# rongzhao-zhang/EfficientQ

Measured on AMD Instinct MI355X. Metric: ptq_calibration_throughput, higher is better.
Workload: dtype i8xi8->i32 (exact) for the Gram systems and per-iteration loss convs of the layers with quantised input, f32/f64 elsewhere

## Files before the change

### efficientq_amd/_lib.py

```python
from __future__ import annotations

import ctypes as C
import os

import torch

_HERE = os.path.dirname(os.path.abspath(__file__))
LIB_PATH = os.path.join(_HERE, "libeffq_hip.so")

EFFQ_OK = 0
_ERR_NAMES = {1: "EFFQ_ERR_ARG", 2: "EFFQ_ERR_HIP", 3: "EFFQ_ERR_WORKSPACE", 4: "EFFQ_ERR_NO_DEVICE",
              5: "EFFQ_ERR_NOT_CONVERGED"}


class EffqError(RuntimeError):
    pass


class Geom(C.Structure):
    _fields_ = [(n, C.c_int32) for n in
                ("N", "C1", "C2", "D", "H", "W", "KD", "KH", "KW", "SD", "SH", "SW", "PD", "PH", "PW")]

    def out_dims(self):
        return ((self.D + 2 * self.PD - self.KD) // self.SD + 1,
                (self.H + 2 * self.PH - self.KH) // self.SH + 1,
                (self.W + 2 * self.PW - self.KW) // self.SW + 1)


class FpState(C.Structure):
    _fields_ = [("alpha", C.c_double), ("alpha_prev", C.c_double), ("sums", C.c_double * 2),
                ("iters", C.c_int32), ("done", C.c_int32)]


FP_STATE_BYTES = C.sizeof(FpState)

_P, _SZ, _I, _F, _D, _LL = C.c_void_p, C.c_size_t, C.c_int, C.c_float, C.c_double, C.c_longlong
_GP = C.POINTER(Geom)
_IP = C.POINTER(C.c_int)
_LLP = C.POINTER(C.c_longlong)


class AdmmRunArgs(C.Structure):
    _fields_ = [("A0", C.c_void_p), ("B0", C.c_void_p), ("W0", C.c_void_p), ("b0", C.c_void_p),
                ("c2", C.c_int32), ("n", C.c_int32), ("has_bias", C.c_int32), ("w_levels", C.c_int32),
                ("iters", C.c_int32), ("rho_period", C.c_int32),
                ("rho", C.c_double), ("rho_max", C.c_double), ("eta", C.c_double), ("tol", C.c_double),
                ("geom", Geom), ("loss_kind", C.c_int32), ("act_levels", C.c_int32),
                ("xq", C.c_void_p), ("xidx", C.c_void_p), ("y_fp", C.c_void_p), ("act_alpha_dev", C.c_void_p),
                ("dual", C.c_void_p), ("wstar", C.c_void_p), ("v", C.c_void_p),
                ("G_ring", C.c_void_p), ("Gq_ring", C.c_void_p), ("b_ring", C.c_void_p), ("state_ring", C.c_void_p),
                ("hist", C.c_void_p), ("err_flag", C.c_void_p),
                ("ainv_pool", C.c_void_p), ("n_ainv", C.c_int32),
                ("prox_ws", C.c_void_p), ("prox_ws_bytes", C.c_size_t),
                ("red_ws", C.c_void_p),
                ("fp_ws", C.c_void_p), ("fp_ws_bytes", C.c_size_t),
                ("fp_pred", C.c_void_p), ("fp_traj_ws", C.c_void_p), ("fp_traj_ws_bytes", C.c_size_t),
                ("inv_ws", C.c_void_p), ("inv_ws_bytes", C.c_size_t),
                ("inv_ws_side", C.c_void_p), ("inv_ws_side_bytes", C.c_size_t),
                ("conv_ws", C.c_void_p), ("conv_ws_bytes", C.c_size_t),
                ("stream_main", C.c_void_p), ("stream_loss", C.c_void_p), ("stream_side", C.c_void_p),
                ("stream_side2", C.c_void_p), ("inv_ws_side2", C.c_void_p), ("inv_ws_side2_bytes", C.c_size_t),
                ("loss_Au", C.c_void_p), ("loss_Bu", C.c_void_p), ("loss_syy", C.c_void_p),
                ("loss_planes", C.c_void_p), ("loss_nplanes", C.c_int32), ("res_ring", C.c_void_p),
                ("channel_wise", C.c_int32), ("alpha_ring", C.c_void_p), ("w_iters_ring", C.c_void_p)]


class ProfRecord(C.Structure):
    _fields_ = [("kind", C.c_int32), ("iter", C.c_int32), ("loss_kind", C.c_int32), ("c2", C.c_int32), ("n", C.c_int32),
                ("geom", Geom), ("ms", C.c_float)]


SIGNATURES = {
    "effq_last_error": (C.c_char_p, []),
    "effq_version": (_I, []),
    "effq_device_count": (_I, [C.POINTER(C.c_int)]),
    "effq_quant_dequant_f32": (_I, [_P, _P, _F, _F, _I, _P, _P, _SZ, _P]),
    "effq_quant_dequant_f64path": (_I, [_P, _P, _D, _D, _I, _P, _P, _P, _SZ, _P]),
    "effq_reduce_ws_bytes": (_SZ, []),
    "effq_abs_sum_f64": (_I, [_P, _SZ, _P, _P, _P]),
    "effq_moments_f64": (_I, [_P, _SZ, _P, _P, _P]),
    "effq_alpha_stats_f64": (_I, [_P, _P, _D, _D, _I, _SZ, _P, _P, _P, _P]),
    "effq_fp_init": (_I, [_P, _P, _P]),
    "effq_fp_update": (_I, [_P, _D, _I, _P]),
    "effq_alpha_fixed_point": (_I, [_P, _SZ, _I, _D, _D, _D, _I, _I, _P, _P, _P]),
    "effq_fp_small_max": (_SZ, []),
    "effq_fixed_point_small": (_I, [_P, _P, _P, _SZ, _I, _D, _D, _D, _I, _P, _P]),
    "effq_fp_coop_max": (_SZ, []),
    "effq_fp_coop_set_spin_limit": (_I, [C.c_uint]),
    "effq_fixed_point_coop": (_I, [_P, _P, _P, _SZ, _I, _D, _D, _D, _I, _P, _P, _P]),
    "effq_fp_bucket_max": (_SZ, []),
    "effq_fp_bucket_ws_bytes": (_SZ, [_SZ]),
    "effq_fixed_point_bucket": (_I, [_P, _P, _P, _SZ, _I, _D, _D, _D, _I, _P, _P, _SZ, _P]),
    "effq_fp_bracket_ws_bytes": (_SZ, [_SZ]),
    "effq_fp_bracket_init": (_I, [_P, _P, _SZ, _I, _I, _P, _SZ, _P]),
    "effq_fp_bracket_run": (_I, [_P, _SZ, _I, _D, _D, _D, _I, _I, _P, _P, _P]),
    "effq_fp_bracket_stats": (_I, [_P, _SZ, _I, _D, _D, _P, _P, _P]),
    "effq_fp_bracket_update": (_I, [_SZ, _I, _D, _D, _D, _I, _P, _P, _P]),
    "effq_fp_traj_max": (_SZ, []),
    "effq_fp_traj_ws_bytes": (_SZ, [_SZ]),
    "effq_spd_inverse_prepare": (_I, [_P]),
    "effq_fp_traj_pred_bytes": (_SZ, []),
    "effq_fixed_point_traj": (_I, [_P, _P, _P, _SZ, _I, _D, _D, _D, _I, _P, _P, _P, _SZ, _P]),
    "effq_fixed_point_bucket_rec": (_I, [_P, _P, _P, _SZ, _I, _D, _D, _D, _I, _P, _P, _SZ, _P, _P]),
    "effq_fixed_point_coop_rec": (_I, [_P, _P, _P, _SZ, _I, _D, _D, _D, _I, _P, _P, _P, _P]),
    "effq_fp_check": (_I, [_P, _P, _P]),
    "effq_fp_channels_max_row": (_I, []),
    "effq_fixed_point_channels": (_I, [_P, _P, _P, _I, _I, _I, _D, _I, _P, _P, _P, _P]),
    "effq_fixed_point_channels_proj": (_I, [_P, _P, _P, _I, _I, _I, _D, _I, _P, _P, _P, _P, _F, _P, _P, _P, _I, _I, _D,
                                            _D, _P]),
    "effq_gram_packed_elems": (_SZ, [_I, _I]),
    "effq_gram_pack": (_I, [_P, _P, _I, _I, _P, _P]),
    "effq_gram_unpack": (_I, [_P, _I, _I, _P, _P, _P]),
    "effq_act_quant_backward": (_I, [_P, _P, _I, _P, _P, _P, _SZ, _P, _P]),
    "effq_att_classes_ws_bytes": (_SZ, []),
    "effq_att_classes": (_I, [_P, _LL, _P, _P, _P, C.POINTER(C.c_int32), _P, _P]),
    "effq_prof_enable": (_I, [_I]),
    "effq_prof_count": (_I, []),
    "effq_prof_read": (_I, [_I, C.POINTER(ProfRecord)]),
    "effq_admm_num_inverses": (_I, [_D, _D, _I, _I]),
    "effq_admm_run": (_I, [C.POINTER(AdmmRunArgs)]),
    "effq_admm_select_best": (_I, [_P, _I, _P, _P, _SZ, _SZ, _P, _P, _P, _P]),
    "effq_gram_ws_bytes": (_SZ, [_GP, _I]),
    "effq_gram_accum": (_I, [_P, _P, _P, _GP, _I, _P, _P, _I, _P, _SZ, _P]),
    "effq_gram_plan_query": (_I, [_GP, _I, _IP, _IP, _IP, _IP, _LLP, _IP, _IP]),
    "effq_gram_i8_supported": (_I, [_GP, _I]),
    "effq_gram_i8_ws_bytes": (_SZ, [_GP, _I]),
    "effq_gram_accum_i8": (_I, [_P, _P, _GP, _I, _P, _I, _P, _P, _P, _I, _LL, _P, _P, _I, _P, _SZ, _P]),
    "effq_gram_accum_i8_unw": (_I, [_P, _P, _GP, _I, _P, _I, _P, _P, _P, _I, _LL, _P, _P, _I, _P, _P, _P, _SZ, _P]),
    "effq_gram_i8_plan_query": (_I, [_GP, _I, _LL, _IP, _IP, _IP, _IP, _IP, _IP]),
    "effq_upsample_trilinear": (_I, [_P, _I, _I, _I, _I, _I, _I, _I, _I, _P, _P]),
    "effq_gram_f64_supported": (_I, [_GP, _I]),
    "effq_gram_f64_ws_bytes": (_SZ, [_GP, _I]),
    "effq_gram_f64": (_I, [_P, _P, _GP, _I, _P, _P, _P, _SZ, _P]),
    "effq_gram_f64_plan_query": (_I, [_GP, _I, _IP, _IP, _IP, _IP]),
    "effq_gram_loss_ws_bytes": (_SZ, [_I]),
    "effq_gram_loss": (_I, [_P, _P, _P, _P, _P, _I, _I, _I, _P, _P, _SZ, _P]),
    "effq_packed_bytes": (_SZ, [_SZ, _I]),
    "effq_pack_levels": (_I, [_P, _SZ, _I, _P, _P]),
    "effq_unpack_levels": (_I, [_P, _SZ, _I, _P, _P]),
    "effq_ainv_ld": (_I, [_I]),
    "effq_fp_bracket_export_words": (_SZ, []),
    "effq_fp_bracket_export": (_I, [_P, _SZ, _P, _P, _SZ, _P]),
    "effq_fp_bracket_rebase": (_I, [_P, _P, _SZ, _P]),
    "effq_fp_bracket_import": (_I, [_P, _SZ, _P, _I, _SZ, _P, _P, _SZ, _P]),
    "effq_admm_uses_traj": (_I, [_SZ, _I]),
    "effq_gram_loss_i8_supported": (_I, [_I, _I, _I, _I]),
    "effq_gram_loss_i8_num_planes": (_I, [C.c_longlong]),
    "effq_gram_loss_i8_planes_bytes": (_SZ, [_I, _I, _I]),
    "effq_gram_loss_i8_prepare": (_I, [_P, _I, _I, _P, _I, _I, _P, _P, _P]),
    "effq_gram_loss_i8_ws_bytes": (_SZ, []),
    "effq_gram_loss_i8": (_I, [_P, _I, _P, _P, _P, _P, _P, _P, _P, _I, _I, _I, _I, _I, _I, _P, _P, _SZ, _P]),
    "effq_spd_inverse_ws_bytes": (_SZ, [_I]),
    "effq_spd_inverse": (_I, [_P, _I, _I, _D, _D, _P, _P, _SZ, _P]),
    "effq_spd_inverse_plan": (_I, [_I, _IP, _IP, _IP]),
    "effq_prox_plan_query": (_I, [_I, _I, _IP, _IP, _IP, _IP]),
    "effq_prox_ws_bytes": (_SZ, [_I, _I]),
    "effq_prox_solve": (_I, [_P, _P, _P, _P, _P, _P, _I, _I, _I, _D, _D, _P, _P, _P, _SZ, _P]),
    "effq_prox_solve_shifted": (_I, [_P, _P, _P, _P, _P, _P, _I, _I, _I, _D, _D, _D, _I, _P, _P, _P, _SZ, _P]),
    "effq_admm_presum": (_I, [_P, _P, _P, _SZ, _P]),
    "effq_admm_project_dual": (_I, [_P, _P, _P, _I, _P, _P, _F, _P, _SZ, _P]),
    "effq_conv_i8_supported": (_I, [_GP, _I, _I]),
    "effq_conv_i8s_supported": (_I, [_GP, _I, _I]),
    "effq_conv_i8s_ws_bytes": (_SZ, [_GP, _I, _I]),
    "conv3d_calib_step_i8s": (_I, [_P, _P, _P, _P, _GP, _P, _I, _P, _I, _I, _P, _P, _SZ, _P]),
    "effq_conv_i8_ws_bytes": (_SZ, [_GP]),
    "conv3d_calib_step_i8": (_I, [_P, _P, _P, _P, _GP, _P, _I, _P, _I, _P, _P, _SZ, _P]),
    "effq_conv_i8_out_supported": (_I, [_GP, _I, _I]),
    "conv3d_quant_forward_i8": (_I, [_P, _P, _P, _P, _P, _GP, _P, _I, _P, _I, _P, _P, _P, _SZ, _P]),
    "effq_conv_ws_bytes": (_SZ, [_GP]),
    "conv3d_quant_calib_step": (_I, [_P, _P, _P, _P, _P, _GP, _P, _I, _P, _P, _P, _SZ, _P]),
    "effq_adam_step": (_I, [_P, _P, _P, _P, _F, _F, _F, _F, _I, _SZ, _P]),
    "effq_window_gather": (_I, [_P, _I, _I, _I, _I, _I, _I, _I, _I, _I, _I, _I, _I, _I, _P, _P]),
    "effq_window_stitch": (_I, [_P, _I, _I, _I, _I, _I, _I, _I, _I, _I, _I, _I, _P, _P]),
    "effq_seg_tallies": (_I, [_P, _P, _I, _LL, _I, _I, _F, _P, _P, _SZ, _P]),
    "effq_seg_labels": (_I, [_P, _I, _I, _LL, _I, _I, _F, _I, _P, _P]),
    "effq_cc_ws_bytes": (_SZ, [_I, _I, _I, _I]),
    "effq_cc_label": (_I, [_P, _I, _I, _I, _I, _I, _P, _P, _P, _SZ, _P]),
    "effq_seg_lesions": (_I, [_P, _P, _I, _I, _I, _I, _I, _I, _F, _I, _P, _P, _SZ, _P]),
    "effq_surf_ws_bytes": (_SZ, [_I, _I, _I, _I]),
    "effq_edt_sq": (_I, [_P, _I, _I, _I, _I, _P, _P, _SZ, _P]),
    "effq_seg_surface": (_I, [_P, _P, _I, _I, _I, _I, _I, _I, _F, _P, _P, _P, _SZ, _P]),
    "effq_surf_mm_ws_bytes": (_SZ, [_I, _I, _I, _I]),
    "effq_edt_sq_mm": (_I, [_P, _I, _I, _I, _I, _F, _F, _F, _P, _P, _SZ, _P]),
    "effq_seg_surface_mm": (_I, [_P, _P, _I, _I, _I, _I, _I, _I, _F, _F, _F, _F, _P, _P, _P, _P, _SZ, _P]),
}

SEG_TALLIES_WS_BYTES = 1024 * 3 * 8 * 4
SEG_TALLIES_MAX_CLASSES = 8
SEG_ARGMAX, SEG_SIGMOID = 0, 1
SEG_FUSE = {None: 0, "agg": 1, "aggressive": 1, "con": 2, "conservative": 2}
SEG_LABEL_RULES = {"argmax": 0, "brats": 1, "rank": 2, "planes": 3}
LESION_CONNECTIVITY = 26
EDT_MAX_LINE = 16382
EDT_MM_MAX_EXTENT = 4096

_lib = None


def load():
    global _lib
    if _lib is not None:
        return _lib
    if not os.path.exists(LIB_PATH):
        raise EffqError(f"{LIB_PATH} is missing: run `python -c 'import __graft_entry__ as g; g.build()'` "
                        f"or `make -C efficientq_amd/csrc` (there is no CPU fallback)")
    lib = C.CDLL(LIB_PATH)
    for name, (res, args) in SIGNATURES.items():
        fn = getattr(lib, name)
        fn.restype, fn.argtypes = res, args
    _lib = lib
    return lib


def check(rc: int, what: str):
    if rc != EFFQ_OK:
        msg = load().effq_last_error().decode(errors="replace")
        raise EffqError(f"{what} failed with {_ERR_NAMES.get(rc, rc)}: {msg}")
```

### efficientq_amd/csrc/admm_run.hip

```cpp
#include <stdlib.h>
#include <algorithm>
#include <vector>
#include "common.h"
#include "internal.h"
#include "project_dual.h"

namespace effq {

struct ProfRec {
  int kind, iter, loss_kind, c2, n;
  effq_geom geom;
  hipEvent_t e0, e1;
};
static thread_local std::vector<ProfRec> g_prof;
static thread_local int g_prof_every = 0;
enum { PROF_PROX = 1, PROF_FIXED_POINT = 2, PROF_PROJECT = 3, PROF_LOSS = 4, PROF_INVERSE = 5, PROF_WAIT = 6 };

struct ProfScope {
  bool on;
  hipStream_t stream;
  ProfRec rec;
  ProfScope(bool enabled, int kind, int iter, const effq_admm_run_args* a, hipStream_t st) : on(enabled), stream(st) {
    if (!on) return;
    rec.kind = kind;
    rec.iter = iter;
    rec.loss_kind = a->loss_kind;
    rec.c2 = a->c2;
    rec.n = a->n;
    rec.geom = a->geom;
    if (hipEventCreate(&rec.e0) != hipSuccess || hipEventCreate(&rec.e1) != hipSuccess) {
      on = false;
      return;
    }
    (void)hipEventRecord(rec.e0, stream);
  }
  void close() {
    if (!on) return;
    (void)hipEventRecord(rec.e1, stream);
    g_prof.push_back(rec);
    on = false;
  }
};

constexpr int ADMM_MAX_RHOS = 16;

struct RhoPlan {
  int count;
  double rho[ADMM_MAX_RHOS];
  int first_iter[ADMM_MAX_RHOS];
  bool shifted_first;
  bool overflow;
};

static RhoPlan plan_rhos(double rho, double rho_max, int iters, int period) {
  RhoPlan p;
  p.count = 0;
  p.overflow = false;
  double r = rho;
  for (int i = 0; i < iters; ++i) {
    if (p.count == 0 || p.rho[p.count - 1] != r) {
      if (p.count == ADMM_MAX_RHOS) {
        p.overflow = true;
        break;
      }
      p.rho[p.count] = r;
      p.first_iter[p.count] = i;
      ++p.count;
    }
    if (i % period == 0) r = (r * 2 <= rho_max) ? r * 2 : rho_max;
  }
  p.shifted_first = p.count > 1 && p.first_iter[1] == 1 && p.rho[1] > p.rho[0];
  return p;
}

static int shift_terms(double rho, double eta, double rho_inv) {
  const double d = rho_inv - rho;
  if (d <= 0) return 1;
  int t = (int)ceil(-26.0 * log(2.0) / log(d / (rho_inv + eta)));
  return t < 2 ? 2 : (t > 64 ? 64 : t);
}

__global__ __launch_bounds__(256) void k_gram_pack(const float* __restrict__ A0, const float* __restrict__ B0, int n, int c2,
                                                   float* __restrict__ buf) {
  const size_t tri = (size_t)n * (n + 1) / 2, nb = (size_t)c2 * n;
  const size_t stride = (size_t)gridDim.x * blockDim.x;
  for (size_t e = (size_t)blockIdx.x * blockDim.x + threadIdx.x; e < (size_t)n * n + nb; e += stride) {
    if (e < (size_t)n * n) {
      const int i = (int)(e / n), j = (int)(e % n);
      if (j >= i) buf[(size_t)i * n - (size_t)i * (i - 1) / 2 + (j - i)] = A0[e];
    } else {
      buf[tri + (e - (size_t)n * n)] = B0[e - (size_t)n * n];
    }
  }
}
__global__ __launch_bounds__(256) void k_gram_unpack(const float* __restrict__ buf, int n, int c2, float* __restrict__ A0,
                                                     float* __restrict__ B0) {
  const size_t tri = (size_t)n * (n + 1) / 2, nb = (size_t)c2 * n;
  const size_t stride = (size_t)gridDim.x * blockDim.x;
  for (size_t e = (size_t)blockIdx.x * blockDim.x + threadIdx.x; e < (size_t)n * n + nb; e += stride) {
    if (e < (size_t)n * n) {
      int i = (int)(e / n), j = (int)(e % n);
      if (j < i) {
        const int t = i;
        i = j;
        j = t;
      }
      A0[e] = buf[(size_t)i * n - (size_t)i * (i - 1) / 2 + (j - i)];
    } else {
      B0[e - (size_t)n * n] = buf[tri + (e - (size_t)n * n)];
    }
  }
}

__global__ __launch_bounds__(256) void k_select_best(const double* __restrict__ hist, int iters,
                                                     const float* __restrict__ G_ring, const float* __restrict__ b_ring,
                                                     size_t nw, size_t nb, float* __restrict__ best_G,
                                                     float* __restrict__ best_b, double* __restrict__ best_out) {
  int bi = 0;
  double bl = hist[0];
  for (int i = 1; i < iters; ++i) {
    const double l = hist[2 * (size_t)i];
    if (l < bl) {
      bl = l;
      bi = i;
    }
  }
  const size_t stride = (size_t)gridDim.x * blockDim.x;
  const size_t t0 = (size_t)blockIdx.x * blockDim.x + threadIdx.x;
  const float* g = G_ring + (size_t)bi * nw;
  for (size_t i = t0; i < nw; i += stride) best_G[i] = g[i];
  if (b_ring != nullptr)
    for (size_t i = t0; i < nb; i += stride) best_b[i] = b_ring[(size_t)bi * nb + i];
  if (t0 == 0) {
    best_out[0] = bl;
    best_out[1] = (double)bi;
  }
}

__global__ __launch_bounds__(256) void k_admm_residuals(const float* __restrict__ wstar, const float* __restrict__ G,
                                                        const float* __restrict__ G0, size_t n, double* __restrict__ res) {
  __shared__ double sh[2][4];
  double a = 0.0, b = 0.0;
  for (size_t i = (size_t)blockIdx.x * blockDim.x + threadIdx.x; i < n; i += (size_t)gridDim.x * blockDim.x) {
    const double p = (double)wstar[i] - (double)G[i], q = (double)G[i] - (double)G0[i];
    a += p * p;
    b += q * q;
  }
  a = wave_sum_f64_dpp(a);
  b = wave_sum_f64_dpp(b);
  const int lane = threadIdx.x & 63, wid = threadIdx.x >> 6;
  if (lane == 0) {
    sh[0][wid] = a;
    sh[1][wid] = b;
  }
  __syncthreads();
  if (threadIdx.x < 2) atomicAdd(res + threadIdx.x, (sh[threadIdx.x][0] + sh[threadIdx.x][1]) + (sh[threadIdx.x][2] + sh[threadIdx.x][3]));
}

struct AdmmPlan {
  int c2, n, has_b;
  size_t nw;
  RhoPlan rhos;
  int first, n_inv;
  size_t ainv_elems;
  bool chan, bucket, traj;
  int traj_after;
  hipStream_t s_main, s_loss, s_side, s_side2;
  bool fork_loss, fork_side, two_sides;
  int side_iter;
  int loss_group;
  float* bm;
  int bm_ld;
};
static int admm_plan(const effq_admm_run_args* a, AdmmPlan* p) {
  EFFQ_CHECK_ARG(a != nullptr);
  EFFQ_CHECK_ARG(a->A0 && a->B0 && a->W0 && a->dual && a->wstar && a->v && a->G_ring && a->state_ring && a->hist &&
                 a->err_flag && a->ainv_pool && a->prox_ws && a->red_ws && a->inv_ws && a->conv_ws && a->y_fp);
  EFFQ_CHECK_ARG(a->c2 > 0 && a->n > 1 && a->iters > 0 && a->rho_period > 0 && a->w_levels >= 2 && a->w_levels <= 256);
  EFFQ_CHECK_ARG((a->has_bias != 0) == (a->b0 != nullptr) && (a->has_bias != 0) == (a->b_ring != nullptr));
  EFFQ_CHECK_ARG((a->loss_kind >= 0 && a->loss_kind <= 2) || a->loss_kind == 4 || a->loss_kind == 5);
  if (a->loss_kind == 4)
    EFFQ_CHECK_ARG(a->loss_Au != nullptr && a->loss_Bu != nullptr && a->loss_syy != nullptr);
  else if (a->loss_kind == 5)
    EFFQ_CHECK_ARG(a->loss_Au != nullptr && a->loss_Bu != nullptr && a->loss_syy != nullptr && a->loss_planes != nullptr &&
                   a->loss_nplanes > 0 && a->Gq_ring != nullptr && a->act_alpha_dev != nullptr &&
                   effq_gram_loss_i8_supported(a->c2, a->n, a->has_bias, a->w_levels));
  else
    EFFQ_CHECK_ARG(a->loss_kind == 0 ? (a->xq != nullptr) : (a->xidx != nullptr && a->Gq_ring != nullptr &&
                                                            a->act_alpha_dev != nullptr));
  p->c2 = a->c2;
  p->n = a->n;
  p->has_b = a->has_bias ? 1 : 0;
  const size_t nw = p->nw = (size_t)p->c2 * (size_t)(p->n - p->has_b);
  EFFQ_CHECK_ARG(nw == (size_t)a->geom.C2 * a->geom.C1 * a->geom.KD * a->geom.KH * a->geom.KW);
  p->chan = a->channel_wise != 0;
  if (p->chan)
    EFFQ_CHECK_ARG((a->loss_kind == 0 || a->loss_kind == 4) && a->alpha_ring != nullptr &&
                   p->n - p->has_b <= effq_fp_channels_max_row());
  if (nw > effq_fp_coop_max()) {
    set_error("admm_run: %zu weights exceed the single-launch fixed points", nw);
    return EFFQ_ERR_ARG;
  }
  constexpr size_t bucket_max = (size_t)1 << 19;
  p->bucket = !p->chan && a->fp_ws != nullptr && a->w_levels <= 16 && nw > 4096 && nw <= bucket_max;
  if (p->bucket && a->fp_ws_bytes < effq_fp_bucket_ws_bytes(nw)) {
    set_error("admm_run: fixed-point workspace %zu < %zu", a->fp_ws_bytes, effq_fp_bucket_ws_bytes(nw));
    return EFFQ_ERR_WORKSPACE;
  }
  p->traj_after = (nw > ((size_t)1 << 20)) ? 30 : 12;
  p->traj = !p->chan && a->fp_pred != nullptr && a->fp_traj_ws != nullptr && effq_admm_uses_traj(nw, a->w_levels) != 0;
  if (p->traj && a->fp_traj_ws_bytes < effq_fp_traj_ws_bytes(nw)) {
    set_error("admm_run: trajectory fixed-point workspace %zu < %zu", a->fp_traj_ws_bytes, effq_fp_traj_ws_bytes(nw));
    return EFFQ_ERR_WORKSPACE;
  }
  p->rhos = plan_rhos(a->rho, a->rho_max, a->iters, a->rho_period);
  EFFQ_CHECK_ARG(!p->rhos.overflow);
  p->first = p->rhos.shifted_first ? 1 : 0;
  p->n_inv = p->rhos.count - p->first;
  EFFQ_CHECK_ARG(a->n_ainv >= p->n_inv);
  p->ainv_elems = (size_t)p->n * (size_t)effq_ainv_ld(p->n);
  p->s_main = as_stream(a->stream_main);
  p->s_loss = a->stream_loss ? as_stream(a->stream_loss) : p->s_main;
  p->s_side = (a->stream_side && a->inv_ws_side) ? as_stream(a->stream_side) : p->s_main;
  p->fork_loss = p->s_loss != p->s_main;
  p->fork_side = p->s_side != p->s_main;
  p->s_side2 = (p->fork_side && a->stream_side2 && a->inv_ws_side2) ? as_stream(a->stream_side2) : p->s_side;
  p->two_sides = p->s_side2 != p->s_side;
  constexpr int SIDE_AFTER_ITERS = 8;
  p->side_iter = p->n_inv <= 1 ? -1 : !p->fork_side ? 0 : std::min(SIDE_AFTER_ITERS, p->rhos.first_iter[p->first + 1] - 1);
  static const int group_gram = getenv("EFFQ_LOSS_GROUP") ? atoi(getenv("EFFQ_LOSS_GROUP")) : 8;
  constexpr int group_conv = 4;
  const int group_size = (a->loss_kind == 4 || a->loss_kind == 5) ? group_gram : group_conv;
  p->loss_group = (p->fork_loss && group_size > 1) ? group_size : 1;
  p->bm = effq_prox_bm(a->prox_ws, p->c2, p->n, &p->bm_ld);
  return EFFQ_OK;
}

struct EventPool {
  std::vector<hipEvent_t>* pool = nullptr;
  size_t used = 0;
  hipError_t open() {
    static thread_local std::vector<std::vector<hipEvent_t>> per_device;
    int dev = 0;
    const hipError_t e = hipGetDevice(&dev);
    if (e == hipSuccess && (int)per_device.size() <= dev) per_device.resize(dev + 1);
    if (e == hipSuccess) pool = &per_device[dev];
    return e;
  }
  hipError_t take(hipEvent_t* ev) {
    if (used == pool->size()) {
      hipEvent_t fresh;
      const hipError_t e = hipEventCreateWithFlags(&fresh, hipEventDisableTiming);
      if (e != hipSuccess) return e;
      pool->push_back(fresh);
    }
    *ev = (*pool)[used++];
    return hipSuccess;
  }
  hipError_t hand_over(hipStream_t from, hipStream_t into, hipEvent_t ev = nullptr) {
    hipError_t e = ev ? hipSuccess : take(&ev);
    if (e == hipSuccess) e = hipEventRecord(ev, from);
    return e == hipSuccess ? hipStreamWaitEvent(into, ev, 0) : e;
  }
};

static int enqueue_later_inverses(const effq_admm_run_args* a, const AdmmPlan& p, EventPool& events, hipEvent_t* ev_inv) {
  for (int r = p.first + 1; r < p.rhos.count; ++r) {
    float* dst = a->ainv_pool + (size_t)(r - p.first) * p.ainv_elems;
    const bool on2 = p.two_sides && ((r - p.first) % 2 == 0);
    hipStream_t sr = on2 ? p.s_side2 : p.s_side;
    void* ws = !p.fork_side ? a->inv_ws : (on2 ? a->inv_ws_side2 : a->inv_ws_side);
    const size_t wsb = !p.fork_side ? a->inv_ws_bytes : (on2 ? a->inv_ws_side2_bytes : a->inv_ws_side_bytes);
    ProfScope ps(g_prof_every > 0, PROF_INVERSE, -1 - r, a, sr);
    const int rc = effq_spd_inverse(a->A0, p.n, p.has_b, p.rhos.rho[r], a->eta, dst, ws, wsb, sr);
    if (rc != EFFQ_OK) return rc;
    ps.close();
    if (p.fork_side) {
      EFFQ_HIP(events.take(&ev_inv[r]));
      EFFQ_HIP(hipEventRecord(ev_inv[r], sr));
    }
  }
  return EFFQ_OK;
}

struct AdmmIter {
  int i;
  double rho, rho_next;
  float dual_div;
  bool use_shift, use_traj, prof;
  bool next_rhs;
  const float* G_prev;
  float *G, *bstar;
  int8_t* Gq;
  effq_fp_state* st;
  const float* parts;
  int parts_n, parts_ld;
};
static AdmmIter admm_iter(const effq_admm_run_args* a, const AdmmPlan& p, int i, double rho, bool use_traj) {
  const bool step = i % a->rho_period == 0, doubles = rho * 2 <= a->rho_max;
  const bool use_shift = p.rhos.shifted_first && i == 0;
  const bool prof = g_prof_every > 0 && !use_shift && (i % g_prof_every) == g_prof_every / 2;
  return AdmmIter{i, rho, !step ? rho : doubles ? rho * 2 : a->rho_max,
                  !step ? 1.0f : doubles ? 2.0f : (float)(a->rho_max / rho), use_shift, use_traj, prof, i + 1 < a->iters,
                  (i == 0) ? a->W0 : a->G_ring + (size_t)(i - 1) * p.nw, a->G_ring + (size_t)i * p.nw,
                  p.has_b ? a->b_ring + (size_t)i * p.c2 : nullptr, a->Gq_ring ? a->Gq_ring + (size_t)i * p.nw : nullptr,
                  a->state_ring + i, nullptr, 1, 0};
}

static int enqueue_prox(const effq_admm_run_args* a, const AdmmPlan& p, AdmmIter* it, const float* Ainv, bool bm_ready) {
  if (!it->use_shift && bm_ready && it->use_traj && p.c2 <= 512)
    return effq_prox_solve_prebuilt_parts(a->B0, Ainv, a->W0, a->b0, it->G_prev, a->dual, p.c2, p.n, p.has_b, it->rho,
                                          a->eta, a->wstar, it->bstar, a->prox_ws, a->prox_ws_bytes, p.s_main,
                                          &it->parts, &it->parts_n, &it->parts_ld);
  if (it->use_shift)
    return effq_prox_solve_shifted(a->B0, a->ainv_pool, a->W0, a->b0, it->G_prev, a->dual, p.c2, p.n, p.has_b, it->rho,
                                   a->eta, p.rhos.rho[1], shift_terms(it->rho, a->eta, p.rhos.rho[1]), a->wstar, it->bstar,
                                   a->prox_ws, a->prox_ws_bytes, p.s_main);
  const auto solve = bm_ready ? effq_prox_solve_prebuilt : effq_prox_solve;
  return solve(a->B0, Ainv, a->W0, a->b0, it->G_prev, a->dual, p.c2, p.n, p.has_b, it->rho, a->eta, a->wstar, it->bstar,
               a->prox_ws, a->prox_ws_bytes, p.s_main);
}

enum class FpKind { channels, traj, bucket, small, coop };
static FpKind fp_kind(const AdmmPlan& p, bool use_traj) {
  if (p.chan) return FpKind::channels;
  if (use_traj) return FpKind::traj;
  if (p.bucket) return FpKind::bucket;
  return p.nw <= effq_fp_small_max() ? FpKind::small : FpKind::coop;
}

static int enqueue_fixed_point(const effq_admm_run_args* a, const AdmmPlan& p, const AdmmIter& it, bool* bm_ready) {
  const int nwrow = p.n - p.has_b;
  const uintptr_t al16 = reinterpret_cast<uintptr_t>(a->v) | reinterpret_cast<uintptr_t>(a->wstar) |
                         reinterpret_cast<uintptr_t>(it.G) | reinterpret_cast<uintptr_t>(a->dual) |
                         (it.next_rhs ? (reinterpret_cast<uintptr_t>(a->W0) | reinterpret_cast<uintptr_t>(p.bm)) : 0);
  const bool vec_ok = (al16 & 15) == 0 && (reinterpret_cast<uintptr_t>(it.Gq) & 3) == 0 && (p.nw % 4) == 0 &&
                      (!it.next_rhs || ((nwrow % 4) == 0 && (p.bm_ld % 4) == 0));
  const FpKind kind = fp_kind(p, it.use_traj);
  const bool fuse_proj = kind == FpKind::channels || (kind == FpKind::small && vec_ok);
  ProjFused pf;
  memset(&pf, 0, sizeof(pf));
  pf.wstar = a->wstar; pf.G = it.G; pf.dual = a->dual; pf.Gq = it.Gq; pf.err_flag = a->err_flag;
  pf.d = 2.0 / (double)(a->w_levels - 1); pf.dual_div = it.dual_div; pf.lm1 = a->w_levels - 1;
  pf.n4 = (unsigned)(p.nw / 4);
  if (it.next_rhs) {
    pf.nx.Bm = p.bm; pf.nx.B0 = a->B0; pf.nx.W0 = a->W0; pf.nx.nwrow = nwrow; pf.nx.n = p.n; pf.nx.ldb = p.bm_ld;
    pf.nx.rho = (float)it.rho_next; pf.nx.eta = (float)a->eta;
  }
  void* rec = p.traj ? a->fp_pred : nullptr;
  const int maxit = 100 * a->w_levels;
  ProfScope p_fp(it.prof, PROF_FIXED_POINT, it.i, a, p.s_main);
  int rc;
  if (kind == FpKind::channels)
    rc = effq_fixed_point_channels_proj(a->wstar, a->dual, a->v, p.c2, nwrow, a->w_levels, a->tol, maxit,
                                        a->alpha_ring + (size_t)it.i * p.c2,
                                        a->w_iters_ring ? a->w_iters_ring + (size_t)it.i * p.c2 : nullptr, a->err_flag,
                                        it.G, it.dual_div, it.next_rhs ? p.bm : nullptr, a->B0, a->W0, p.n, p.bm_ld,
                                        it.rho_next, a->eta, p.s_main);
  else if (kind == FpKind::traj && it.parts != nullptr)
    rc = effq_fixed_point_traj_parts(it.parts, it.parts_n, it.parts_ld, p.c2, nwrow, p.has_b, a->dual, a->wstar, it.bstar,
                                     a->v, a->w_levels, -1.0, 1.0, a->tol, maxit, it.st, a->fp_pred, a->fp_traj_ws,
                                     a->fp_traj_ws_bytes, p.s_main);
  else if (kind == FpKind::traj)
    rc = effq_fixed_point_traj(a->wstar, a->dual, a->v, p.nw, a->w_levels, -1.0, 1.0, a->tol, maxit, it.st, a->fp_pred,
                               a->fp_traj_ws, a->fp_traj_ws_bytes, p.s_main);
  else if (kind == FpKind::bucket)
    rc = effq_fixed_point_bucket_rec(a->wstar, a->dual, a->v, p.nw, a->w_levels, -1.0, 1.0, a->tol, maxit, it.st, a->fp_ws,
                                     a->fp_ws_bytes, rec, p.s_main);
  else if (kind == FpKind::small)
    rc = effq_fixed_point_small_fused(a->wstar, a->dual, a->v, p.nw, a->w_levels, -1.0, 1.0, a->tol, maxit, it.st,
                                      fuse_proj ? &pf : nullptr, p.s_main);
  else
    rc = effq_fixed_point_coop_rec(a->wstar, a->dual, a->v, p.nw, a->w_levels, -1.0, 1.0, a->tol, maxit, it.st, a->red_ws,
                                   rec, p.s_main);
  if (rc != EFFQ_OK) return rc;
  p_fp.close();
  *bm_ready = it.next_rhs;
  if (fuse_proj) return EFFQ_OK;
  ProfScope p_pr(it.prof, PROF_PROJECT, it.i, a, p.s_main);
  if (it.next_rhs)
    rc = effq_project_dual_next(a->v, a->wstar, it.st, a->w_levels, it.G, a->dual, it.dual_div, it.Gq, p.nw, a->err_flag,
                                p.bm, a->B0, a->W0, nwrow, p.n, p.bm_ld, it.rho_next, a->eta, p.s_main);
  else
    rc = effq_project_dual_checked(a->v, a->wstar, it.st, a->w_levels, it.G, a->dual, it.dual_div, it.Gq, p.nw,
                                   a->err_flag, p.s_main);
  if (rc != EFFQ_OK) return rc;
  p_pr.close();
  return EFFQ_OK;
}

static int enqueue_losses(const effq_admm_run_args* a, const AdmmPlan& p, int j0, int i) {
  const int step = a->loss_kind == 5 ? 16 : 1;
  for (int j = j0; j <= i; j += step) {
    const int cnt = (i - j + 1 < step) ? (i - j + 1) : step;
    const float* Gj = a->G_ring + (size_t)j * p.nw;
    const int8_t* Gqj = a->Gq_ring ? a->Gq_ring + (size_t)j * p.nw : nullptr;
    const float* bj = p.has_b ? a->b_ring + (size_t)j * p.c2 : nullptr;
    const effq_fp_state* stj = a->state_ring + j;
    double* sq = a->hist + 2 * (size_t)j;
    const bool prof = g_prof_every > 0 && (a->loss_kind == 5 ? (j / p.loss_group) % 2 == 1 :
                      !(p.rhos.shifted_first && j == 0) && (j % g_prof_every) == g_prof_every / 2);
    ProfScope p_loss(prof, PROF_LOSS, j, a, p.s_loss);
    int rc;
    if (a->loss_kind == 5)
      rc = effq_gram_loss_i8(a->loss_planes, a->loss_nplanes, a->loss_Au, a->loss_Bu, a->loss_syy, Gqj, bj, stj,
                             a->act_alpha_dev, a->act_levels, a->w_levels, p.c2, p.n, p.has_b, cnt, sq, a->conv_ws,
                             a->conv_ws_bytes, p.s_loss);
    else if (a->loss_kind == 1)
      rc = conv3d_calib_step_i8(a->xidx, Gqj, bj, a->y_fp, &a->geom, a->act_alpha_dev, a->act_levels, stj, a->w_levels,
                                sq, a->conv_ws, a->conv_ws_bytes, p.s_loss);
    else if (a->loss_kind == 2)
      rc = conv3d_calib_step_i8s(a->xidx, Gqj, bj, a->y_fp, &a->geom, a->act_alpha_dev, a->act_levels, stj, a->w_levels,
                                 j == 0 ? 1 : 0, sq, a->conv_ws, a->conv_ws_bytes, p.s_loss);
    else if (a->loss_kind == 4)
      rc = effq_gram_loss(a->loss_Au, a->loss_Bu, a->loss_syy, Gj, bj, p.c2, p.n, p.has_b, sq, a->conv_ws,
                          a->conv_ws_bytes, p.s_loss);
    else
      rc = conv3d_quant_calib_step(a->xq, Gj, bj, a->y_fp, nullptr, &a->geom, nullptr, 0, sq, nullptr, a->conv_ws,
                                   a->conv_ws_bytes, p.s_loss);
    if (rc != EFFQ_OK) return rc;
    p_loss.close();
  }
  return EFFQ_OK;
}

}
using namespace effq;

extern "C" {

int effq_admm_uses_traj(size_t nw, int w_levels) {
  constexpr int traj_levels = 4;
  constexpr size_t traj_min = 65536;
  return (w_levels <= traj_levels && nw >= traj_min && nw <= effq_fp_traj_max()) ? 1 : 0;
}

int effq_admm_num_inverses(double rho, double rho_max, int iters, int period) {
  if (!(rho > 0.0) || iters <= 0 || period <= 0) return -1;
  const RhoPlan p = plan_rhos(rho, rho_max, iters, period);
  if (p.overflow) return -1;
  return p.count - (p.shifted_first ? 1 : 0);
}

int effq_admm_run(const effq_admm_run_args* a) {
  AdmmPlan p;
  if (const int rc = admm_plan(a, &p); rc != EFFQ_OK) return rc;
  constexpr int LOSS_EVENTS = 4;
  EventPool events;
  EFFQ_HIP(events.open());
  hipEvent_t ev_inv[ADMM_MAX_RHOS] = {}, ev_loss[LOSS_EVENTS] = {};
  EFFQ_HIP(hipMemsetAsync(a->dual, 0, p.nw * sizeof(float), p.s_main));
  if (a->res_ring != nullptr) EFFQ_HIP(hipMemsetAsync(a->res_ring, 0, 2 * (size_t)a->iters * sizeof(double), p.s_main));
  if (p.traj) EFFQ_HIP(hipMemsetAsync(a->fp_pred, 0, effq_fp_traj_pred_bytes(), p.s_main));
  if (p.fork_side && p.n_inv > 1) {
    hipEvent_t ev_fork;
    EFFQ_HIP(events.take(&ev_fork));
    EFFQ_HIP(hipEventRecord(ev_fork, p.s_main));
    EFFQ_HIP(hipStreamWaitEvent(p.s_side, ev_fork, 0));
    if (p.two_sides) EFFQ_HIP(hipStreamWaitEvent(p.s_side2, ev_fork, 0));
  }
  ProfScope p_inv(g_prof_every > 0, PROF_INVERSE, -1, a, p.s_main);
  if (const int rc = effq_spd_inverse(a->A0, p.n, p.has_b, p.rhos.rho[p.first], a->eta, a->ainv_pool, a->inv_ws,
                                      a->inv_ws_bytes, p.s_main); rc != EFFQ_OK)
    return rc;
  p_inv.close();
  if (p.fork_loss)
    for (int e = 0; e < LOSS_EVENTS; ++e) EFFQ_HIP(events.take(&ev_loss[e]));
  bool bm_ready = false;
  const float* Ainv = nullptr;
  int k = 0;
  int cur = -1;
  int loss_next = 0;
  for (int i = 0; i < a->iters; ++i) {
    if (k + 1 < p.rhos.count && p.rhos.first_iter[k + 1] == i) ++k;
    if (i == p.side_iter)
      if (const int rc = enqueue_later_inverses(a, p, events, ev_inv); rc != EFFQ_OK) return rc;
    AdmmIter it = admm_iter(a, p, i, p.rhos.rho[k], p.traj && i - p.rhos.first_iter[k] >= p.traj_after);
    if (!it.use_shift && cur != k) {
      EFFQ_CHECK_ARG(p.rhos.rho[k] == p.rhos.rho[k]);
      if (p.fork_side && ev_inv[k] != nullptr) {
        ProfScope p_wait(g_prof_every > 0, PROF_WAIT, i, a, p.s_main);
        EFFQ_HIP(hipStreamWaitEvent(p.s_main, ev_inv[k], 0));
        p_wait.close();
      }
      Ainv = a->ainv_pool + (size_t)(k - p.first) * p.ainv_elems;
      cur = k;
    }
    ProfScope p_prox(it.prof, PROF_PROX, i, a, p.s_main);
    if (const int rc = enqueue_prox(a, p, &it, Ainv, bm_ready); rc != EFFQ_OK) return rc;
    p_prox.close();
    if (const int rc = enqueue_fixed_point(a, p, it, &bm_ready); rc != EFFQ_OK) return rc;
    if (a->res_ring != nullptr) {
      const size_t nb = std::min<size_t>((p.nw + 1023) / 1024, 256);
      hipLaunchKernelGGL(k_admm_residuals, dim3((unsigned)nb), dim3(256), 0, p.s_main, a->wstar, it.G, it.G_prev, p.nw,
                         a->res_ring + 2 * (size_t)i);
      EFFQ_LAUNCH_CHECK();
    }
    if (!p.fork_loss || (i + 1) % p.loss_group == 0 || i + 1 == a->iters) {
      if (p.fork_loss) EFFQ_HIP(events.hand_over(p.s_main, p.s_loss, ev_loss[(i / p.loss_group) % LOSS_EVENTS]));
      if (const int rc = enqueue_losses(a, p, loss_next, i); rc != EFFQ_OK) return rc;
      loss_next = i + 1;
    }
  }
  ProfScope p_join(g_prof_every > 0 && (p.fork_loss || p.fork_side), PROF_WAIT, a->iters, a, p.s_main);
  if (p.fork_loss) EFFQ_HIP(events.hand_over(p.s_loss, p.s_main));
  if (p.fork_side && p.n_inv > 1) EFFQ_HIP(events.hand_over(p.s_side, p.s_main));
  if (p.fork_side && p.n_inv > 1 && p.two_sides) EFFQ_HIP(events.hand_over(p.s_side2, p.s_main));
  p_join.close();
  return EFFQ_OK;
}

size_t effq_gram_packed_elems(int n, int c2) {
  return (n > 0 && c2 > 0) ? (size_t)n * (n + 1) / 2 + (size_t)c2 * n : 0;
}

int effq_gram_pack(const float* A0, const float* B0, int n, int c2, float* buf, void* stream) {
  EFFQ_CHECK_ARG(A0 && B0 && buf && n > 0 && c2 > 0);
  size_t blocks = ((size_t)n * n + (size_t)c2 * n + 255) / 256;
  if (blocks > 8192) blocks = 8192;
  hipLaunchKernelGGL(k_gram_pack, dim3((unsigned)blocks), dim3(256), 0, as_stream(stream), A0, B0, n, c2, buf);
  EFFQ_LAUNCH_CHECK();
  return EFFQ_OK;
}

int effq_gram_unpack(const float* buf, int n, int c2, float* A0, float* B0, void* stream) {
  EFFQ_CHECK_ARG(A0 && B0 && buf && n > 0 && c2 > 0);
  size_t blocks = ((size_t)n * n + (size_t)c2 * n + 255) / 256;
  if (blocks > 8192) blocks = 8192;
  hipLaunchKernelGGL(k_gram_unpack, dim3((unsigned)blocks), dim3(256), 0, as_stream(stream), buf, n, c2, A0, B0);
  EFFQ_LAUNCH_CHECK();
  return EFFQ_OK;
}

int effq_prof_enable(int every) {
  for (ProfRec& r : g_prof) {
    (void)hipEventDestroy(r.e0);
    (void)hipEventDestroy(r.e1);
  }
  g_prof.clear();
  g_prof_every = every > 0 ? every : 0;
  return EFFQ_OK;
}

int effq_prof_count(void) { return (int)g_prof.size(); }

int effq_prof_read(int i, effq_prof_record* out) {
  EFFQ_CHECK_ARG(out != nullptr && i >= 0 && i < (int)g_prof.size());
  const ProfRec& r = g_prof[(size_t)i];
  float ms = 0.0f;
  EFFQ_HIP(hipEventElapsedTime(&ms, r.e0, r.e1));
  out->kind = r.kind;
  out->iter = r.iter;
  out->loss_kind = r.loss_kind;
  out->c2 = r.c2;
  out->n = r.n;
  out->geom = r.geom;
  out->ms = ms;
  return EFFQ_OK;
}

int effq_admm_select_best(const double* hist, int iters, const float* G_ring, const float* b_ring, size_t nw, size_t nb,
                          float* best_G, float* best_b, double* best_out, void* stream) {
  EFFQ_CHECK_ARG(hist && G_ring && best_G && best_out && iters > 0 && nw > 0);
  EFFQ_CHECK_ARG((b_ring == nullptr) == (best_b == nullptr));
  size_t blocks = (nw + 255) / 256;
  if (blocks > 1024) blocks = 1024;
  hipLaunchKernelGGL(k_select_best, dim3((unsigned)blocks), dim3(256), 0, as_stream(stream), hist, iters, G_ring, b_ring,
                     nw, nb, best_G, best_b, best_out);
  EFFQ_LAUNCH_CHECK();
  return EFFQ_OK;
}

}
```

### efficientq_amd/csrc/internal.h

```cpp
#pragma once
#include "common.h"

namespace effq {
struct ProjFused;
}

extern "C" {

int effq_fixed_point_small_fused(const float* a, const float* b, float* v_out, size_t n, int levels, double lo, double hi,
                                 double tol, int max_iter, effq_fp_state* state_dev, const effq::ProjFused* pf_in,
                                 void* stream);
int effq_project_dual_checked(const float* v, const float* wstar, const effq_fp_state* state_dev, int levels, float* G,
                              float* dual, float dual_div, int8_t* Gq_out, size_t n, int32_t* err_flag_dev,
                              void* stream);
int effq_project_dual_next(const float* v, const float* wstar, const effq_fp_state* state_dev, int levels, float* G,
                           float* dual, float dual_div, int8_t* Gq_out, size_t n, int32_t* err_flag_dev, float* Bm,
                           const float* B0, const float* W0, int nwrow, int nb0, int ldb, double rho_next, double eta,
                           void* stream);

float* effq_prox_bm(void* ws, int c2, int n, int* ldb);
int effq_prox_solve_prebuilt(const float* B0, const float* Ainv, const float* W0, const float* b0, const float* G,
                             const float* dual, int c2, int n, int has_bias, double rho, double eta, float* wstar,
                             float* bstar, void* ws, size_t ws_bytes, void* stream);
int effq_prox_solve_prebuilt_parts(const float* B0, const float* Ainv, const float* W0, const float* b0, const float* G,
                                   const float* dual, int c2, int n, int has_bias, double rho, double eta, float* wstar,
                                   float* bstar, void* ws, size_t ws_bytes, void* stream, const float** part_out,
                                   int* nsplit_out, int* ldp_out);

int effq_fixed_point_traj_parts(const float* part, int nsplit, int ldp, int c2, int nwrow, int has_bias, const float* dual,
                                float* wstar_out, float* bstar_out, float* v_out, int levels, double lo, double hi, double tol,
                                int max_iter, effq_fp_state* state_dev, void* pred_dev, void* ws, size_t ws_bytes,
                                void* stream);

}
```

### efficientq_amd/csrc/solve.hip

```cpp
#include <cstdlib>
#include <vector>
#include "common.h"
#include "internal.h"

namespace effq {

typedef float f32x16 __attribute__((ext_vector_type(16)));
typedef double f64x4 __attribute__((ext_vector_type(4)));
typedef float f32x4 __attribute__((ext_vector_type(4)));

static inline int round_up(int v, int m) { return (v + m - 1) / m * m; }

constexpr int NBK = 64;
constexpr int LDA_S = 66;
constexpr int LDB_S = 80;

__global__ __launch_bounds__(256) void k_build_a64(const float* __restrict__ A0, int n, int npad, int has_bias,
                                                   double rho, double eta, double* __restrict__ A64) {
  const size_t tot = (size_t)npad * npad;
  const size_t stride = (size_t)gridDim.x * blockDim.x;
  for (size_t e = (size_t)blockIdx.x * blockDim.x + threadIdx.x; e < tot; e += stride) {
    const int i = (int)(e / npad), j = (int)(e % npad);
    double v = 0.0;
    if (i < n && j < n) {
// ... 635 lines not shown
      v.w = v.w + rho * (g.w - du.w);
      if (wprev != nullptr) {
        const float4 wp = *reinterpret_cast<const float4*>(wprev + wi);
        v.x = v.x + shift * wp.x;
        v.y = v.y + shift * wp.y;
        v.z = v.z + shift * wp.z;
        v.w = v.w + shift * wp.w;
      }
    } else if (r < c2 && k == nw && has_bias) {
      v.x = B0[(size_t)r * n + k] + eta * b0[r];
    }
    *reinterpret_cast<float4*>(out + k) = v;
  }
}

__global__ __launch_bounds__(256) void k_prox_reduce4(const float* __restrict__ part, int ldp, int nsplit, int c2, int n,
                                                      int has_bias, float* __restrict__ wstar, float* __restrict__ bstar) {
  __builtin_amdgcn_s_setprio(2);

  const int r = blockIdx.y;
  const int nw = n - has_bias;
  const size_t tot = (size_t)c2 * ldp;
  const float* row = part + (size_t)r * ldp;
  for (int k = (blockIdx.x * blockDim.x + threadIdx.x) * 4; k < ldp; k += gridDim.x * blockDim.x * 4) {
    if (k >= n) continue;
    float4 v = *reinterpret_cast<const float4*>(row + k);
    for (int z = 1; z < nsplit; ++z) {
      const float4 t = *reinterpret_cast<const float4*>(row + (size_t)z * tot + k);
      v.x += t.x;
      v.y += t.y;
      v.z += t.z;
      v.w += t.w;
    }
    if (k < nw)
      *reinterpret_cast<float4*>(wstar + (size_t)r * nw + k) = v;
    else
      bstar[r] = v.x;
  }
}

constexpr int PBK = 32, PLD = PBK + 4;

template <int MT, int WM, int WN, int NTN>
__global__ __launch_bounds__(256) void k_prox_gemm(const float* __restrict__ Bm, int ldb, const float* __restrict__ Ainv,
                                                   int lda, int n, int c2, int has_bias, float* __restrict__ wstar,
                                                   float* __restrict__ bstar, float* __restrict__ part, int ldp) {
  __builtin_amdgcn_s_setprio(2);

  constexpr int BM = 32 * MT * WM, BN = 32 * WN * NTN;
  constexpr int NA = BM * 8 / 256, NB = BN * 8 / 256;
  static_assert(WM * WN == 4 && NA >= 1 && NB >= 1, "4 waves");
  __shared__ __attribute__((aligned(16))) float As[BM * PLD];
  __shared__ __attribute__((aligned(16))) float Bs[BN * PLD];
  const int tid = threadIdx.x, lane = tid & 63, wid = tid >> 6;
  const int li = lane & 31, lh = lane >> 5;
  const int wm = wid / WN, wn = wid % WN;
  const int row0 = blockIdx.y * BM, col0 = blockIdx.x * BN;

  f32x16 acc[MT][NTN];
#pragma unroll
  for (int m = 0; m < MT; ++m)
#pragma unroll
    for (int t = 0; t < NTN; ++t)
#pragma unroll
      for (int r = 0; r < 16; ++r) acc[m][t][r] = 0.0f;

  f32x4 ra[NA], rb[NB];
  const float* pa[NA];
  const float* pb[NB];
#pragma unroll
  for (int q = 0; q < NA; ++q) {
    const int u = tid + q * 256, r = u >> 3, c4 = u & 7;
    pa[q] = Bm + (size_t)(row0 + r) * ldb + c4 * 4;
  }
#pragma unroll
  for (int q = 0; q < NB; ++q) {
    const int u = tid + q * 256, r = u >> 3, c4 = u & 7;
    pb[q] = Ainv + (size_t)min(col0 + r, n - 1) * lda + c4 * 4;
  }
#define EFFQ_PROX_FETCH(k0)                                                         \
  {                                                                                 \
    _Pragma("unroll") for (int q = 0; q < NA; ++q)                                  \
        ra[q] = *reinterpret_cast<const f32x4*>(pa[q] + (k0));                      \
    _Pragma("unroll") for (int q = 0; q < NB; ++q)                                  \
        rb[q] = *reinterpret_cast<const f32x4*>(pb[q] + (k0));                      \
  }
  const int nkt = ldb / PBK;
  const int kt0 = (int)(((long long)nkt * blockIdx.z) / gridDim.z);
  const int nk = (int)(((long long)nkt * (blockIdx.z + 1)) / gridDim.z);
  EFFQ_PROX_FETCH(kt0 * PBK)
  for (int kt = kt0; kt < nk; ++kt) {
    lds_barrier();
#pragma unroll
    for (int q = 0; q < NA; ++q) {
      const int u = tid + q * 256;
      *reinterpret_cast<f32x4*>(&As[(u >> 3) * PLD + (u & 7) * 4]) = ra[q];
    }
#pragma unroll
    for (int q = 0; q < NB; ++q) {
      const int u = tid + q * 256;
      *reinterpret_cast<f32x4*>(&Bs[(u >> 3) * PLD + (u & 7) * 4]) = rb[q];
    }
    lds_barrier();
    EFFQ_PROX_FETCH(min(kt + 1, nk - 1) * PBK)
    __builtin_amdgcn_sched_barrier(0);
#pragma unroll
    for (int q = 0; q < 4; ++q) {
      f32x4 a[MT], b[NTN];
#pragma unroll
      for (int m = 0; m < MT; ++m)
        a[m] = *reinterpret_cast<const f32x4*>(&As[((wm * MT + m) * 32 + li) * PLD + q * 8 + 4 * lh]);
#pragma unroll
      for (int t = 0; t < NTN; ++t)
        b[t] = *reinterpret_cast<const f32x4*>(&Bs[((wn * NTN + t) * 32 + li) * PLD + q * 8 + 4 * lh]);
#pragma unroll
      for (int m = 0; m < MT; ++m)
#pragma unroll
        for (int t = 0; t < NTN; ++t)
#pragma unroll
          for (int e = 0; e < 4; ++e)
            acc[m][t] = __builtin_amdgcn_mfma_f32_32x32x2f32(a[m][e], b[t][e], acc[m][t], 0, 0, 0);
    }
  }
#undef EFFQ_PROX_FETCH
  const int nw = n - has_bias;
  if (gridDim.z > 1) {
    float* P = part + (size_t)blockIdx.z * c2 * ldp;
#pragma unroll
    for (int m = 0; m < MT; ++m)
#pragma unroll
      for (int t = 0; t < NTN; ++t) {
        const int col = col0 + (wn * NTN + t) * 32 + li;
#pragma unroll
        for (int r = 0; r < 16; ++r) {
          const int row = row0 + (wm * MT + m) * 32 + (r & 3) + 8 * (r >> 2) + 4 * lh;
          if (row < c2 && col < n) P[(size_t)row * ldp + col] = acc[m][t][r];
        }
      }
    return;
  }
#pragma unroll
  for (int m = 0; m < MT; ++m)
#pragma unroll
    for (int t = 0; t < NTN; ++t) {
      const int col = col0 + (wn * NTN + t) * 32 + li;
#pragma unroll
      for (int r = 0; r < 16; ++r) {
        const int row = row0 + (wm * MT + m) * 32 + (r & 3) + 8 * (r >> 2) + 4 * lh;
        if (row < c2 && col < n) {
          if (col < nw)
            wstar[(size_t)row * nw + col] = acc[m][t][r];
          else
            bstar[row] = acc[m][t][r];
        }
      }
    }
}


typedef __bf16 bf16x8 __attribute__((ext_vector_type(8)));
typedef __bf16 bf16x4 __attribute__((ext_vector_type(4)));
constexpr int B3_K = 16;
constexpr int B3_LD = B3_K + 8;

__device__ __forceinline__ void split3(const f32x4 v, bf16x4& p0, bf16x4& p1, bf16x4& p2) {
#pragma unroll
  for (int e = 0; e < 4; ++e) {
    const __bf16 b0 = (__bf16)v[e];
    const float r1 = v[e] - (float)b0;
    const __bf16 b1 = (__bf16)r1;
    const float r2 = r1 - (float)b1;
    p0[e] = b0;
    p1[e] = b1;
    p2[e] = (__bf16)r2;
  }
}

template <int BM, int BN, int WM, int WN>
__global__ __launch_bounds__(512) void k_prox_gemm_b3(const float* __restrict__ Bm, int ldb, const float* __restrict__ Ainv,
                                                      int lda, int n, int c2, int has_bias, float* __restrict__ wstar,
                                                      float* __restrict__ bstar, float* __restrict__ part, int ldp) {
  __builtin_amdgcn_s_setprio(2);
  constexpr int MT = BM / WM / 32, NT = BN / WN / 32;
  constexpr int NA = BM * 4 / 512, NB = BN * 4 / 512;
  constexpr int STAGE = 3 * (BM + BN) * B3_LD;
  static_assert(WM * WN == 8 && MT >= 1 && NT >= 1 && NA >= 1 && NB >= 1, "8 waves");
  extern __shared__ __attribute__((aligned(16))) unsigned char b3_lds[];
  __bf16* lds = reinterpret_cast<__bf16*>(b3_lds);
  const int tid = threadIdx.x, lane = tid & 63, wid = tid >> 6;
  const int li = lane & 31, lh = lane >> 5;
  const int wm = wid / WN, wn = wid % WN;
  const int row0 = blockIdx.y * BM, col0 = blockIdx.x * BN;

  f32x16 acc[MT][NT];
#pragma unroll
  for (int m = 0; m < MT; ++m)
#pragma unroll
    for (int t = 0; t < NT; ++t)
#pragma unroll
      for (int r = 0; r < 16; ++r) acc[m][t][r] = 0.0f;

  f32x4 ra[NA], rb[NB];
  const float* pa[NA];
  const float* pb[NB];
#pragma unroll
  for (int q = 0; q < NA; ++q) {
    const int u = tid + q * 512, r = u >> 2, c4 = u & 3;
    pa[q] = Bm + (size_t)(row0 + r) * ldb + c4 * 4;
  }
#pragma unroll
  for (int q = 0; q < NB; ++q) {
    const int u = tid + q * 512, r = u >> 2, c4 = u & 3;
    pb[q] = Ainv + (size_t)min(col0 + r, n - 1) * lda + c4 * 4;
  }
#define EFFQ_B3_FETCH(k0)                                                           \
  {                                                                                 \
    _Pragma("unroll") for (int q = 0; q < NA; ++q)                                  \
        ra[q] = *reinterpret_cast<const f32x4*>(pa[q] + (k0));                      \
    _Pragma("unroll") for (int q = 0; q < NB; ++q)                                  \
        rb[q] = *reinterpret_cast<const f32x4*>(pb[q] + (k0));                      \
  }
#define EFFQ_B3_STORE(stage)                                                                        \
  {                                                                                                 \
    __bf16* As_ = lds + (stage) * STAGE;                                                            \
    __bf16* Bs_ = As_ + 3 * BM * B3_LD;                                                             \
    _Pragma("unroll") for (int q = 0; q < NA; ++q) {                                                \
      const int u = tid + q * 512, off = (u >> 2) * B3_LD + (u & 3) * 4;                            \
      bf16x4 p0, p1, p2;                                                                            \
      split3(ra[q], p0, p1, p2);                                                                    \
      *reinterpret_cast<bf16x4*>(&As_[off]) = p0;                                                   \
      *reinterpret_cast<bf16x4*>(&As_[BM * B3_LD + off]) = p1;                                      \
      *reinterpret_cast<bf16x4*>(&As_[2 * BM * B3_LD + off]) = p2;                                  \
    }                                                                                               \
    _Pragma("unroll") for (int q = 0; q < NB; ++q) {                                                \
      const int u = tid + q * 512, off = (u >> 2) * B3_LD + (u & 3) * 4;                            \
      bf16x4 p0, p1, p2;                                                                            \
      split3(rb[q], p0, p1, p2);                                                                    \
      *reinterpret_cast<bf16x4*>(&Bs_[off]) = p0;                                                   \
      *reinterpret_cast<bf16x4*>(&Bs_[BN * B3_LD + off]) = p1;                                      \
      *reinterpret_cast<bf16x4*>(&Bs_[2 * BN * B3_LD + off]) = p2;                                  \
    }                                                                                               \
  }
  const int nkt = ldb / B3_K;
  const int kt0 = (int)(((long long)nkt * blockIdx.z) / gridDim.z);
  const int nk = (int)(((long long)nkt * (blockIdx.z + 1)) / gridDim.z);
  EFFQ_B3_FETCH(kt0 * B3_K)
  EFFQ_B3_STORE(0)
  EFFQ_B3_FETCH(min(kt0 + 1, nk - 1) * B3_K)
  lds_barrier();
  for (int kt = kt0; kt < nk; ++kt) {
    const int st = (kt - kt0) & 1;
    if (kt + 1 < nk) EFFQ_B3_STORE(st ^ 1)
    EFFQ_B3_FETCH(min(kt + 2, nk - 1) * B3_K)
    const __bf16* As = lds + st * STAGE;
    const __bf16* Bs = As + 3 * BM * B3_LD;
    bf16x8 a[MT][3], b[NT][3];
#pragma unroll
    for (int m = 0; m < MT; ++m)
#pragma unroll
      for (int p = 0; p < 3; ++p)
        a[m][p] = *reinterpret_cast<const bf16x8*>(&As[p * BM * B3_LD + ((wm * MT + m) * 32 + li) * B3_LD + 8 * lh]);
#pragma unroll
    for (int t = 0; t < NT; ++t)
#pragma unroll
      for (int p = 0; p < 3; ++p)
        b[t][p] = *reinterpret_cast<const bf16x8*>(&Bs[p * BN * B3_LD + ((wn * NT + t) * 32 + li) * B3_LD + 8 * lh]);
#pragma unroll
    for (int m = 0; m < MT; ++m)
#pragma unroll
      for (int t = 0; t < NT; ++t) {
        acc[m][t] = __builtin_amdgcn_mfma_f32_32x32x16_bf16(a[m][0], b[t][2], acc[m][t], 0, 0, 0);
        acc[m][t] = __builtin_amdgcn_mfma_f32_32x32x16_bf16(a[m][1], b[t][1], acc[m][t], 0, 0, 0);
        acc[m][t] = __builtin_amdgcn_mfma_f32_32x32x16_bf16(a[m][2], b[t][0], acc[m][t], 0, 0, 0);
        acc[m][t] = __builtin_amdgcn_mfma_f32_32x32x16_bf16(a[m][0], b[t][1], acc[m][t], 0, 0, 0);
        acc[m][t] = __builtin_amdgcn_mfma_f32_32x32x16_bf16(a[m][1], b[t][0], acc[m][t], 0, 0, 0);
        acc[m][t] = __builtin_amdgcn_mfma_f32_32x32x16_bf16(a[m][0], b[t][0], acc[m][t], 0, 0, 0);
      }
    lds_barrier();
  }
#undef EFFQ_B3_FETCH
#undef EFFQ_B3_STORE
  const int nw = n - has_bias;
  float* P = (gridDim.z > 1) ? part + (size_t)blockIdx.z * c2 * ldp : nullptr;
#pragma unroll
  for (int m = 0; m < MT; ++m)
#pragma unroll
    for (int t = 0; t < NT; ++t) {
      const int col = col0 + (wn * NT + t) * 32 + li;
#pragma unroll
      for (int r = 0; r < 16; ++r) {
        const int row = row0 + (wm * MT + m) * 32 + (r & 3) + 8 * (r >> 2) + 4 * lh;
        if (row < c2 && col < n) {
          if (P != nullptr)
            P[(size_t)row * ldp + col] = acc[m][t][r];
          else if (col < nw)
            wstar[(size_t)row * nw + col] = acc[m][t][r];
          else
            bstar[row] = acc[m][t][r];
        }
      }
    }
}

__global__ __launch_bounds__(256) void k_prox_reduce(const float* __restrict__ part, int ldp, int nsplit, int c2, int n,
                                                     int has_bias, float* __restrict__ wstar, float* __restrict__ bstar) {
  const size_t tot = (size_t)c2 * ldp, stride = (size_t)gridDim.x * blockDim.x;
  const int nw = n - has_bias;
  for (size_t e = (size_t)blockIdx.x * blockDim.x + threadIdx.x; e < tot; e += stride) {
    const int row = (int)(e / ldp), col = (int)(e % ldp);
    if (col >= n) continue;
    float v = part[e];
    for (int z = 1; z < nsplit; ++z) v += part[(size_t)z * tot + e];
    if (col < nw)
      wstar[(size_t)row * nw + col] = v;
    else
      bstar[row] = v;
  }
}

struct ProxPlan { int variant, gx, gy, nsplit, c2p, ldb; };
static ProxPlan prox_plan(int c2, int n) {
  ProxPlan p;
  p.c2p = (c2 > 128) ? round_up(c2, 256) : (c2 > 64) ? 128 : round_up(c2, 32);
  p.ldb = round_up(n, 32);
  if (p.c2p >= 128 && n >= 1024) {
    p.variant = 5; p.gx = (n + 255) / 256; p.gy = p.c2p / 256;
    if (p.c2p == 128) { p.variant = 7; p.gx = (n + 127) / 128; p.gy = 1; }
    const int tiles5 = p.gx * p.gy, nkt5 = p.ldb / B3_K;
    int s5 = (256 + tiles5 / 2) / tiles5;
    if (s5 > nkt5 / 16) s5 = nkt5 / 16;
    if (s5 < 1) s5 = 1;
    p.nsplit = s5;
    return p;
  }
  if (p.c2p >= 256) { p.variant = 0; p.gx = (n + 63) / 64; p.gy = p.c2p / 256; }
  else if (p.c2p == 128) { p.variant = 1; p.gx = (n + 63) / 64; p.gy = 1; }
  else if (p.c2p == 64) { p.variant = 2; p.gx = (n + 63) / 64; p.gy = 1; }
  else { p.variant = 3; p.gx = (n + 127) / 128; p.gy = 1; }
  const int tiles = p.gx * p.gy, nkt = p.ldb / PBK;
  int s = (440 + tiles - 1) / tiles;
  if (s > nkt / 6) s = nkt / 6;
  if (s > 16) s = 16;
  if (s < 1) s = 1;
  if (p.variant == 0) {
    const int smax = s > 1 ? 16 : 1;
    double best = -1.0;
    for (int c = 1; c <= smax && c <= nkt / 6; ++c) {
      const int wgs = tiles * c, rounds = (wgs + 767) / 768;
      const double score = (double)wgs / (768.0 * rounds) - 0.01 * c;
      if (score > best) { best = score; s = c; }
    }
  }
  p.nsplit = s;
  return p;
}

}

using namespace effq;

extern "C" {

static size_t gj64_aux_doubles(size_t npad) { return 2 * (size_t)NBK * npad + 2 * NBK * NBK; }

constexpr int GJ_WIDE_MIN_BLOCKS = 100;
static bool gj_takes_wide(int nblk) { return nblk >= GJ_WIDE_MIN_BLOCKS; }
static int gj_wide_pivot(int nblk) { return (nblk >= 100) ? effq::WB : 2; }

size_t effq_spd_inverse_ws_bytes(int n) {
  if (n <= 0) return 0;
  const size_t npad = (size_t)round_up(n, NBK);
  size_t d = npad * npad + gj64_aux_doubles(npad);
  if (gj_takes_wide((int)(npad / NBK))) {
    const size_t ldx = (size_t)round_up((int)npad, BG_T);
    d = npad * npad + 2 * (size_t)WK * ldx + (size_t)WK * WK + gj64_aux_doubles(WK);
  }
  return d * sizeof(double) + 256;
}

int effq_ainv_ld(int n) { return n > 0 ? round_up(n, 32) : 0; }

static int gj64_sweep(double* A64, int npad, double* aux, hipStream_t st) {
  const int nblk = npad / NBK;
  double* XT = aux;
  double* NZ = XT + (size_t)NBK * npad;
  double* Dinv = NZ + (size_t)NBK * npad;
  const size_t lds = (size_t)(NBK * LDA_S + NBK * LDB_S) * sizeof(double);
  for (int k = 0; k < nblk; ++k) {
    const int kb = k * NBK;
    double* Dk = Dinv + (size_t)(k & 1) * NBK * NBK;
    double* Dn = Dinv + (size_t)((k + 1) & 1) * NBK * NBK;
    if (k == 0) hipLaunchKernelGGL(k_gj_diag, dim3(1), dim3(GJD_T), 0, st, A64, npad, kb, Dk);
    hipLaunchKernelGGL(k_gj_panel, dim3(nblk), dim3(256), lds, st, A64, npad, kb, Dk, NZ, XT);
    if (nblk > 1)
      hipLaunchKernelGGL(k_gj_trail_sym, dim3((nblk + GJ_CT - 1) / GJ_CT, nblk + 1), dim3(256), 0, st, A64, npad, kb, NZ,
                         XT, Dn);
    EFFQ_LAUNCH_CHECK();
  }
  return EFFQ_OK;
}

struct GjWideCtx {
  int dev;
  hipStream_t caller, helper;
  hipEvent_t e1, e2;
};
static thread_local std::vector<GjWideCtx> g_gj_ctx;

static int gj_wide_ctx(hipStream_t caller, GjWideCtx** out) {
  int dev = 0;
  EFFQ_HIP(hipGetDevice(&dev));
  for (GjWideCtx& c : g_gj_ctx)
    if (c.dev == dev && c.caller == caller) {
      *out = &c;
      return EFFQ_OK;
    }
  GjWideCtx c;
  c.dev = dev;
  c.caller = caller;
  int prio = 0;
  if (hipStreamGetPriority(caller, &prio) != hipSuccess) prio = 0;
  EFFQ_HIP(hipStreamCreateWithPriority(&c.helper, hipStreamNonBlocking, prio));
  EFFQ_HIP(hipEventCreateWithFlags(&c.e1, hipEventDisableTiming));
  EFFQ_HIP(hipEventCreateWithFlags(&c.e2, hipEventDisableTiming));
  g_gj_ctx.push_back(c);
  *out = &g_gj_ctx.back();
  return EFFQ_OK;
}

static int gj_wide_sweep(double* A64, int npad, double* aux, hipStream_t st) {
  const int nblk = npad / NBK;
  const int WB = gj_wide_pivot(nblk);
  const size_t ldx = (size_t)round_up(npad, BG_T);
  double* NZT = aux;
  double* XTW = NZT + (size_t)WK * ldx;
  double* Dw = XTW + (size_t)WK * ldx;
  double* aux64 = Dw + (size_t)WK * WK;
  const int nK = (nblk + WB - 1) / WB, nm = (nblk + 1) / 2;
  GjWideCtx* ctx = nullptr;
  if (nK > 1) {
    const int rc = gj_wide_ctx(st, &ctx);
    if (rc != EFFQ_OK) return rc;
  }
  hipStream_t s2 = ctx ? ctx->helper : st;
  const size_t lds = (size_t)(NBK * LDA_S + NBK * LDB_S) * sizeof(double);
  const size_t pf_lds = (size_t)(2 * NBK * PF_LD + 2 * (NBK + 1)) * sizeof(double);
  auto pivot_block = [&](int k0, int mk, int kdim, hipStream_t s) -> int {
    GjBig g;
    memset(&g, 0, sizeof(g));
    g.Cin = A64; g.ldin = (size_t)npad;
    g.Cout = Dw; g.ldout = (size_t)mk * NBK; g.orow = k0 * NBK; g.ocol = k0 * NBK;
    g.NZT = NZT; g.XTW = XTW; g.ldx = ldx; g.kdim = kdim; g.nblk = nblk;
    g.i0m = k0 / 2; g.j0m = k0 / 2;
    g.skip_lo = g.skip_hi = -1; g.la_lo = g.la_hi = -1;
    if (WB == 2) {
      hipLaunchKernelGGL(k_gj_pivot_fused, dim3(1), dim3(1024), pf_lds, s, A64, npad, k0, mk, NZT, XTW, ldx, kdim, Dw);
      EFFQ_LAUNCH_CHECK();
      return EFFQ_OK;
    }
    const int span = (mk + 1) / 2;
    hipLaunchKernelGGL(k_gj_big, dim3(span, span), dim3(256), 0, s, g);
    EFFQ_LAUNCH_CHECK();
    const int rc = gj64_sweep(Dw, mk * NBK, aux64, s);
    if (rc != EFFQ_OK) return rc;
    hipLaunchKernelGGL(k_mirror_blocks, dim3(64), dim3(256), 0, s, Dw, mk * NBK);
    EFFQ_LAUNCH_CHECK();
    return EFFQ_OK;
  };
  {
    const int rc = pivot_block(0, nblk < WB ? nblk : WB, 0, st);
    if (rc != EFFQ_OK) return rc;
  }
  for (int K = 0; K < nK; ++K) {
    const int kb0 = K * WB, m = (nblk - kb0 < WB) ? nblk - kb0 : WB;
    const int kn0 = kb0 + WB, mn = (K + 1 < nK) ? ((nblk - kn0 < WB) ? nblk - kn0 : WB) : 0;
    hipLaunchKernelGGL(k_gj_panel_w, dim3(nblk, m), dim3(256), lds, st, A64, npad, kb0, m, Dw, NZT, XTW, ldx);
    EFFQ_LAUNCH_CHECK();
    if (ctx) {
      EFFQ_HIP(hipEventRecord(ctx->e1, st));
      EFFQ_HIP(hipStreamWaitEvent(s2, ctx->e1, 0));
    }
    hipLaunchKernelGGL(k_gj_wback_w, dim3(nblk, m), dim3(256), 0, s2, A64, npad, kb0, m, Dw, NZT, ldx);
    EFFQ_LAUNCH_CHECK();
    if (mn > 0) {
      const int rc = pivot_block(kn0, mn, m * NBK, s2);
      if (rc != EFFQ_OK) return rc;
    }
    if (nblk > m) {
      GjBig g;
      memset(&g, 0, sizeof(g));
      g.Cin = A64; g.ldin = (size_t)npad;
      g.Cout = A64; g.ldout = (size_t)npad; g.orow = 0; g.ocol = 0;
      g.NZT = NZT; g.XTW = XTW; g.ldx = ldx; g.kdim = m * NBK; g.nblk = nblk;
      g.i0m = 0; g.j0m = 0;
      g.skip_lo = kb0; g.skip_hi = kb0 + m;
      g.la_lo = mn > 0 ? kn0 : -1; g.la_hi = mn > 0 ? kn0 + mn : -1;
      hipLaunchKernelGGL(k_gj_big, dim3(nm, nm), dim3(256), 0, st, g);
      EFFQ_LAUNCH_CHECK();
    }
    if (ctx) {
      EFFQ_HIP(hipEventRecord(ctx->e2, s2));
      EFFQ_HIP(hipStreamWaitEvent(st, ctx->e2, 0));
    }
  }
  return EFFQ_OK;
}

int effq_spd_inverse_prepare(void* stream) {
  GjWideCtx* ctx = nullptr;
  return gj_wide_ctx(as_stream(stream), &ctx);
}

int effq_spd_inverse(const float* A0, int n, int has_bias, double rho, double eta, float* Ainv, void* ws,
                     size_t ws_bytes, void* stream) {
  EFFQ_CHECK_ARG(A0 && Ainv && ws && n > 0);
  EFFQ_CHECK_ARG(eta > 0.0 && rho >= 0.0);
  if (ws_bytes < effq_spd_inverse_ws_bytes(n)) {
    set_error("spd_inverse: workspace %zu < required %zu", ws_bytes, effq_spd_inverse_ws_bytes(n));
    return EFFQ_ERR_WORKSPACE;
  }
  const int npad = round_up(n, NBK);
  double* A64 = reinterpret_cast<double*>(ws);
  double* aux = A64 + (size_t)npad * npad;
  hipStream_t st = as_stream(stream);
  {
    size_t nb = ((size_t)npad * npad + 255) / 256;
    if (nb > 8192) nb = 8192;
    hipLaunchKernelGGL(k_build_a64, dim3((unsigned)nb), dim3(256), 0, st, A0, n, npad, has_bias, rho, eta, A64);
    EFFQ_LAUNCH_CHECK();
  }
  const size_t lds = (size_t)(NBK * LDA_S + NBK * LDB_S) * sizeof(double);
  EFFQ_HIP(raise_lds_limit<k_gj_panel>(lds));
  EFFQ_HIP(raise_lds_limit<k_gj_panel_w>(lds));
  EFFQ_HIP(raise_lds_limit<k_gj_pivot_fused>((2 * NBK * PF_LD + 2 * (NBK + 1)) * sizeof(double)));
  const int rc = gj_takes_wide(npad / NBK) ? gj_wide_sweep(A64, npad, aux, st) : gj64_sweep(A64, npad, aux, st);
  if (rc != EFFQ_OK) return rc;
  {
    const int lda = effq_ainv_ld(n);
    size_t nb = ((size_t)n * lda + 255) / 256;
    if (nb > 8192) nb = 8192;
    hipLaunchKernelGGL(k_a64_to_f32, dim3((unsigned)nb), dim3(256), 0, st, A64, n, npad, Ainv, lda);
    EFFQ_LAUNCH_CHECK();
  }
  return EFFQ_OK;
}

int effq_spd_inverse_plan(int n, int* wide, int* nblk, int* pivot_blocks) {
  EFFQ_CHECK_ARG(n > 0 && wide && nblk && pivot_blocks);
  const int nb = round_up(n, NBK) / NBK;
  *wide = gj_takes_wide(nb) ? 1 : 0;
  *nblk = nb;
  *pivot_blocks = *wide ? (nb + gj_wide_pivot(nb) - 1) / gj_wide_pivot(nb) : nb;
  return EFFQ_OK;
}

int effq_prox_plan_query(int c2, int n, int* variant, int* gx, int* gy, int* nsplit) {
  EFFQ_CHECK_ARG(c2 > 0 && n > 0 && variant && gx && gy && nsplit);
  const ProxPlan p = prox_plan(c2, n);
  *variant = p.variant;
  *gx = p.gx;
  *gy = p.gy;
  *nsplit = p.nsplit;
  return EFFQ_OK;
}

size_t effq_prox_ws_bytes(int c2, int n) {
  if (c2 <= 0 || n <= 0) return 0;
  const ProxPlan p = prox_plan(c2, n);
  return ((size_t)p.c2p + (p.nsplit > 1 ? (size_t)p.nsplit * c2 : 0)) * p.ldb * sizeof(float) + 256;
}

static int prox_solve_impl(const float* B0, const float* Ainv, const float* W0, const float* b0, const float* G,
                           const float* dual, int c2, int n, int has_bias, double rho, double eta, double shift,
                           int nterms, float* wstar, float* bstar, void* ws, size_t ws_bytes, void* stream,
                           bool prebuilt = false, const float** part_out = nullptr, int* nsplit_out = nullptr,
                           int* ldp_out = nullptr) {
  EFFQ_CHECK_ARG(B0 && Ainv && W0 && G && dual && wstar && ws && c2 > 0 && n > 0 && nterms >= 1);
  EFFQ_CHECK_ARG(!has_bias || (b0 != nullptr && bstar != nullptr));
  if (ws_bytes < effq_prox_ws_bytes(c2, n)) {
    set_error("prox_solve: workspace %zu < required %zu", ws_bytes, effq_prox_ws_bytes(c2, n));
    return EFFQ_ERR_WORKSPACE;
  }
  const ProxPlan pl = prox_plan(c2, n);
  const int c2p = pl.c2p, ldb = pl.ldb;
  const int lda = effq_ainv_ld(n);
  float* Bm = reinterpret_cast<float*>(ws);
  float* part = Bm + (size_t)c2p * ldb;
  hipStream_t st = as_stream(stream);
  for (int term = 0; term < nterms; ++term) {
    if (!(prebuilt && term == 0)) {
      const int nw = n - (has_bias ? 1 : 0);
      if ((nw % 4) == 0) {
        const unsigned bx = (unsigned)((ldb / 4 + 255) / 256);
        hipLaunchKernelGGL(k_build_b4, dim3(bx, (unsigned)c2p), dim3(256), 0, st, B0, W0, b0, G, dual, c2, n,
                           has_bias ? 1 : 0, (float)rho, (float)eta, Bm, ldb, (term > 0) ? wstar : nullptr, (float)shift);
      } else {
        size_t nb = ((size_t)c2p * ldb + 255) / 256;
        if (nb > 4096) nb = 4096;
        hipLaunchKernelGGL(k_build_b, dim3((unsigned)nb), dim3(256), 0, st, B0, W0, b0, G, dual, c2, n, has_bias ? 1 : 0,
                           (float)rho, (float)eta, Bm, ldb, c2p, (term > 0) ? wstar : nullptr, (float)shift);
      }
      EFFQ_LAUNCH_CHECK();
    }
    const dim3 grid(pl.gx, pl.gy, pl.nsplit);
#define EFFQ_PROX_LAUNCH(MT, WM, WN, NTN)                                                                              \
  hipLaunchKernelGGL((k_prox_gemm<MT, WM, WN, NTN>), grid, dim3(256), 0, st, Bm, ldb, Ainv, lda, n, c2, has_bias ? 1 : 0, \
                     wstar, bstar, part, ldb)
    if (pl.variant == 5 || pl.variant == 7) {
      const size_t lds5 = (size_t)2 * 3 * (256 + 256) * B3_LD * sizeof(__bf16);
      const size_t lds7 = (size_t)2 * 3 * (128 + 128) * B3_LD * sizeof(__bf16);
      EFFQ_HIP((raise_lds_limit<k_prox_gemm_b3<256, 256, 4, 2>>(lds5)));
      EFFQ_HIP((raise_lds_limit<k_prox_gemm_b3<128, 128, 2, 4>>(lds7)));
      if (pl.variant == 5)
        hipLaunchKernelGGL((k_prox_gemm_b3<256, 256, 4, 2>), grid, dim3(512), lds5, st, Bm, ldb, Ainv, lda, n, c2,
                           has_bias ? 1 : 0, wstar, bstar, part, ldb);
      else
        hipLaunchKernelGGL((k_prox_gemm_b3<128, 128, 2, 4>), grid, dim3(512), lds7, st, Bm, ldb, Ainv, lda, n, c2,
                           has_bias ? 1 : 0, wstar, bstar, part, ldb);
    } else
    switch (pl.variant) {
      case 0: EFFQ_PROX_LAUNCH(2, 4, 1, 2); break;
      case 1: EFFQ_PROX_LAUNCH(1, 4, 1, 2); break;
      case 2: EFFQ_PROX_LAUNCH(1, 2, 2, 1); break;
      default: EFFQ_PROX_LAUNCH(1, 1, 4, 1); break;
    }
#undef EFFQ_PROX_LAUNCH
    EFFQ_LAUNCH_CHECK();
    if (part_out != nullptr) {
      *part_out = (pl.nsplit > 1) ? part : nullptr;
      *nsplit_out = pl.nsplit;
      *ldp_out = ldb;
    } else if (pl.nsplit > 1) {
      const int nw = n - (has_bias ? 1 : 0);
      if ((nw % 4) == 0) {
        const unsigned bx = (unsigned)((ldb / 4 + 255) / 256);
        hipLaunchKernelGGL(k_prox_reduce4, dim3(bx, (unsigned)c2), dim3(256), 0, st, part, ldb, pl.nsplit, c2, n,
                           has_bias ? 1 : 0, wstar, bstar);
      } else {
        size_t nb = ((size_t)c2 * ldb + 255) / 256;
        if (nb > 2048) nb = 2048;
        hipLaunchKernelGGL(k_prox_reduce, dim3((unsigned)nb), dim3(256), 0, st, part, ldb, pl.nsplit, c2, n,
                           has_bias ? 1 : 0, wstar, bstar);
      }
      EFFQ_LAUNCH_CHECK();
    }
  }
  return EFFQ_OK;
}

int effq_prox_solve(const float* B0, const float* Ainv, const float* W0, const float* b0, const float* G,
                    const float* dual, int c2, int n, int has_bias, double rho, double eta, float* wstar, float* bstar,
                    void* ws, size_t ws_bytes, void* stream) {
  return prox_solve_impl(B0, Ainv, W0, b0, G, dual, c2, n, has_bias, rho, eta, 0.0, 1, wstar, bstar, ws, ws_bytes,
                         stream);
}

float* effq_prox_bm(void* ws, int c2, int n, int* ldb) {
  *ldb = prox_plan(c2, n).ldb;
  return reinterpret_cast<float*>(ws);
}
int effq_prox_solve_prebuilt(const float* B0, const float* Ainv, const float* W0, const float* b0, const float* G,
                             const float* dual, int c2, int n, int has_bias, double rho, double eta, float* wstar,
                             float* bstar, void* ws, size_t ws_bytes, void* stream) {
  return prox_solve_impl(B0, Ainv, W0, b0, G, dual, c2, n, has_bias, rho, eta, 0.0, 1, wstar, bstar, ws, ws_bytes,
                         stream, true);
}

int effq_prox_solve_prebuilt_parts(const float* B0, const float* Ainv, const float* W0, const float* b0, const float* G,
                                   const float* dual, int c2, int n, int has_bias, double rho, double eta, float* wstar,
                                   float* bstar, void* ws, size_t ws_bytes, void* stream, const float** part_out,
                                   int* nsplit_out, int* ldp_out) {
  EFFQ_CHECK_ARG(part_out && nsplit_out && ldp_out);
  return prox_solve_impl(B0, Ainv, W0, b0, G, dual, c2, n, has_bias, rho, eta, 0.0, 1, wstar, bstar, ws, ws_bytes,
                         stream, true, part_out, nsplit_out, ldp_out);
}

int effq_prox_solve_shifted(const float* B0, const float* Ainv, const float* W0, const float* b0, const float* G,
                            const float* dual, int c2, int n, int has_bias, double rho, double eta, double rho_inv,
                            int nterms, float* wstar, float* bstar, void* ws, size_t ws_bytes, void* stream) {
  EFFQ_CHECK_ARG(rho_inv >= rho && rho > 0.0 && eta >= 0.0);
  return prox_solve_impl(B0, Ainv, W0, b0, G, dual, c2, n, has_bias, rho, eta, rho_inv - rho, nterms, wstar, bstar, ws,
                         ws_bytes, stream);
}

}
```

### efficientq_amd/hip_ops.py

```python
from __future__ import annotations

import ctypes as C
import math
from typing import Optional, Tuple

import torch

from . import _lib
from ._lib import Geom, check

ADMM_TOL = 1e-5
FP_BRACKET_MIN = 1 << 18
DP_GATHER_AFTER = 4
DP_GATHER_MAX_BYTES = 128 << 20


def _ptr(t: Optional[torch.Tensor]):
    return None if t is None else C.c_void_p(t.data_ptr())


def to_ndhwc(x: torch.Tensor) -> torch.Tensor:
    return x.permute(0, 2, 3, 4, 1).contiguous()


# ... 248 lines not shown
            batch = min(2 * batch, 256)

    def fp_bracket_diagnostics(self):
        ws = self._ws["fp_bracket"]
        f = ws[:256].view(torch.float64).cpu()
        i = ws[:256].view(torch.int64).cpu()
        return {"blo": float(f[0]), "bhi": float(f[1]), "src": int(i[7]), "G": int(i[10]), "per": int(i[11]),
                "escapes": int(i[12]), "narrowings": int(i[13]), "visited": int(i[14]), "list_total": int(i[15]),
                "density": float(f[17]), "widen": int(i[20]), "base": int(i[21]), "z_total": int(i[22])}

    def weight_fixed_point(self, wstar, dual, v, levels: int, state, guess: int = 16):
        n = wstar.numel()
        if n <= self.lib.effq_fp_small_max():
            check(self.lib.effq_fixed_point_small(_ptr(wstar), _ptr(dual), _ptr(v), n, levels, -1.0, 1.0, ADMM_TOL,
                                                  100 * levels, _ptr(state), self.stream), "effq_fixed_point_small")
            return None
        if n <= self.lib.effq_fp_coop_max():
            check(self.lib.effq_fixed_point_coop(_ptr(wstar), _ptr(dual), _ptr(v), n, levels, -1.0, 1.0, ADMM_TOL,
                                                 100 * levels, _ptr(state), _ptr(self._red_ws), self.stream),
                  "effq_fixed_point_coop")
            return None
        self.admm_presum(wstar, dual, v)
        _, it, _ = self.fit_scale(v, levels, -1.0, 1.0, guess_iters=guess, state=state)
        return it

    def fixed_point_bucket(self, a, b, v, levels: int, state, lo: float = -1.0, hi: float = 1.0):
        n = a.numel()
        ws = self._workspace("fp_bucket", self.lib.effq_fp_bucket_ws_bytes(n))
        check(self.lib.effq_fixed_point_bucket(_ptr(a), _ptr(b), _ptr(v), n, levels, lo, hi, ADMM_TOL, 100 * levels,
                                               _ptr(state), _ptr(ws), ws.numel(), self.stream),
              "effq_fixed_point_bucket")

    def new_fp_pred(self) -> torch.Tensor:
        return torch.zeros(self.lib.effq_fp_traj_pred_bytes(), dtype=torch.uint8, device=self.device)

    def fixed_point_traj(self, a, b, v, levels: int, state, pred, lo: float = -1.0, hi: float = 1.0):
        n = a.numel()
        ws = self._workspace("fp_traj", self.lib.effq_fp_traj_ws_bytes(n))
        check(self.lib.effq_fixed_point_traj(_ptr(a), _ptr(b), _ptr(v), n, levels, lo, hi, ADMM_TOL, 100 * levels,
                                             _ptr(state), _ptr(pred), _ptr(ws), ws.numel(), self.stream),
              "effq_fixed_point_traj")

    def fixed_point_bucket_rec(self, a, b, v, levels: int, state, pred, lo: float = -1.0, hi: float = 1.0):
        n = a.numel()
        ws = self._workspace("fp_bucket", self.lib.effq_fp_bucket_ws_bytes(n))
        check(self.lib.effq_fixed_point_bucket_rec(_ptr(a), _ptr(b), _ptr(v), n, levels, lo, hi, ADMM_TOL, 100 * levels,
                                                   _ptr(state), _ptr(ws), ws.numel(), _ptr(pred), self.stream),
              "effq_fixed_point_bucket_rec")

    def fixed_point_coop_rec(self, a, b, v, levels: int, state, pred, lo: float = -1.0, hi: float = 1.0):
        check(self.lib.effq_fixed_point_coop_rec(_ptr(a), _ptr(b), _ptr(v), a.numel(), levels, lo, hi, ADMM_TOL,
                                                 100 * levels, _ptr(state), _ptr(self._red_ws), _ptr(pred), self.stream),
              "effq_fixed_point_coop_rec")

    @staticmethod
    def read_fp_pred(pred: torch.Tensor):
        i32 = pred[:16].view(torch.int32).cpu()
        f = pred[16:16 + 8 * 40].view(torch.float64).cpu()
        i64 = pred[16 + 8 * 40:16 + 8 * 45].view(torch.int64).cpu()
        fn = pred[16 + 8 * 45:16 + 8 * 53].view(torch.float64).cpu()
        j64 = pred[16 + 8 * 53:16 + 8 * 63].view(torch.int64).cpu()
        K = int(i32[0])
        return {"K": K, "e": int(i32[1]), "lo": f[0:8].tolist(), "hi": f[8:16].tolist(), "eps": f[16:24].tolist(),
                "eps_n": fn.tolist(), "calls": int(i64[0]), "warm_iters": int(i64[1]), "full_iters": int(i64[2]),
                "listed": int(i64[3]), "list_max": int(i64[4]), "ring_iters": int(j64[0]), "ring_listed": int(j64[1]),
                "trace_us": [(int(j64[2 + k]) - int(j64[2])) / 100.0 for k in range(5)],
                "mean_us_phase1_setup_loop": [int(j64[7 + k]) / 100.0 / max(int(i64[0]), 1) for k in range(3)]}

    def fp_check(self, state, err_flag):
        check(self.lib.effq_fp_check(_ptr(state), _ptr(err_flag), self.stream), "effq_fp_check")

    def gram(self, x_ndhwc: torch.Tensor, att: Optional[torch.Tensor], y_ndhwc: torch.Tensor, geom: Geom,
             has_bias: bool, A0: Optional[torch.Tensor] = None, B0: Optional[torch.Tensor] = None):
        x = self._f32(x_ndhwc)
        y = self._f32(y_ndhwc)
        a = self._f32(att) if att is not None else None
        _check_shapes(geom, x, y=y, att=a)
        n = geom.C1 * geom.KD * geom.KH * geom.KW + int(has_bias)
        acc = int(A0 is not None)
        if A0 is not None and (tuple(A0.shape) != (n, n) or tuple(B0.shape) != (geom.C2, n)):
            raise _lib.EffqError("gram: A0/B0 shapes do not match the geometry")
        if A0 is None:
            A0 = torch.empty(n, n, dtype=torch.float32, device=self.device)
            B0 = torch.empty(geom.C2, n, dtype=torch.float32, device=self.device)
        need = self.lib.effq_gram_ws_bytes(C.byref(geom), int(has_bias))
        ws = self._workspace("gram", need)
        check(self.lib.effq_gram_accum(_ptr(x), _ptr(a), _ptr(y), C.byref(geom), int(has_bias), _ptr(A0), _ptr(B0),
                                       acc, _ptr(ws), ws.numel(), self.stream), "effq_gram_accum")
        return A0, B0

    def gram_plan(self, geom: Geom, has_bias: bool) -> dict:
        vec, nb, npairs, nsplit, fold, fin = (C.c_int() for _ in range(6))
        vps = C.c_longlong()
        check(self.lib.effq_gram_plan_query(C.byref(geom), int(has_bias), C.byref(vec), C.byref(nb), C.byref(npairs),
                                            C.byref(nsplit), C.byref(vps), C.byref(fold), C.byref(fin)),
              "effq_gram_plan_query")
        return dict(vec=bool(vec.value), NB=nb.value, npairs=npairs.value, nsplit=nsplit.value, vox_per_split=vps.value,
                    fold=fold.value, finish_blocks=fin.value)

    def gram_i8_plan(self, geom: Geom, ncls: int = 1, n_list: int = 0) -> dict:
        out = [C.c_int() for _ in range(6)]
        check(self.lib.effq_gram_i8_plan_query(C.byref(geom), int(ncls), int(n_list), *[C.byref(o) for o in out]),
              "effq_gram_i8_plan_query")
        return dict(zip(("NB", "NBX", "npairs", "nchunks", "cps", "nsplit"), (o.value for o in out)))

    def gram_f64_plan(self, geom: Geom, has_bias: bool) -> dict:
        out = [C.c_int() for _ in range(4)]
        check(self.lib.effq_gram_f64_plan_query(C.byref(geom), int(has_bias), *[C.byref(o) for o in out]),
              "effq_gram_f64_plan_query")
        return dict(zip(("nchunk", "grid", "ntiles", "tpw"), (o.value for o in out)))

    def gram_i8_supported(self, geom: Geom, act_levels: int) -> bool:
        return bool(self.lib.effq_gram_i8_supported(C.byref(geom), int(act_levels)))

    GRAM_I8_MAX_CLASSES = 16

    def att_classes(self, att: Optional[torch.Tensor]):
        if att is None:
            return (None, None, None, 1)
        key = (att.data_ptr(), att.numel(), att._version)
        hit = self._att_cache.get(key)
        if hit is not None:
            return hit[1]
        flat = self._f32(att).reshape(-1)
        V = flat.numel()
        lst = torch.empty(V + 128 * self.GRAM_I8_MAX_CLASSES, dtype=torch.int32, device=flat.device)
        chunk_cls = torch.empty(V // 128 + self.GRAM_I8_MAX_CLASSES, dtype=torch.int32, device=flat.device)
        cls_w = torch.empty(self.GRAM_I8_MAX_CLASSES, dtype=torch.float32, device=flat.device)
        info = (C.c_int32 * 3)()
        ws = self._workspace("att_cls", self.lib.effq_att_classes_ws_bytes())
        check(self.lib.effq_att_classes(_ptr(flat), V, _ptr(lst), _ptr(chunk_cls), _ptr(cls_w), info, _ptr(ws),
                                        self.stream), "effq_att_classes")
        k, n_list, overflow = int(info[0]), int(info[1]), int(info[2])
        res = None if overflow else (lst[:n_list], chunk_cls[: n_list // 128], cls_w[:k], k)
        if len(self._att_cache) > 16:
            self._att_cache.clear()
        self._att_cache[key] = (att, res)
        return res

    def gram_i8(self, xidx_ndhwc: torch.Tensor, att_cls, y_ndhwc: torch.Tensor, geom: Geom, has_bias: bool,
                act_alpha: torch.Tensor, act_levels: int, A0: Optional[torch.Tensor] = None,
                B0: Optional[torch.Tensor] = None, unweighted: bool = False):
        if xidx_ndhwc.dtype != torch.uint8 or not xidx_ndhwc.is_contiguous():
            raise _lib.EffqError("gram_i8 wants contiguous uint8 level ids")
        y = self._f32(y_ndhwc)
        _check_shapes(geom, xidx_ndhwc, y=y)
        lst, chunk_cls, cls_w, ncls = att_cls
        if lst is not None:
            od, oh, ow = geom.out_dims()
            if (int(lst.numel()) < geom.N * od * oh * ow or lst.numel() % 128 or
                    chunk_cls.numel() * 128 != lst.numel() or cls_w.numel() != ncls):
                raise _lib.EffqError("gram_i8: voxel list does not match the output volume")
        n = geom.C1 * geom.KD * geom.KH * geom.KW + int(has_bias)
        acc = int(A0 is not None)
        if A0 is not None and (tuple(A0.shape) != (n, n) or tuple(B0.shape) != (geom.C2, n)):
            raise _lib.EffqError("gram_i8: A0/B0 shapes do not match the geometry")
        if A0 is None:
            A0 = torch.empty(n, n, dtype=torch.float32, device=self.device)
            B0 = torch.empty(geom.C2, n, dtype=torch.float32, device=self.device)
        al = self._f32(act_alpha.reshape(1))
        ws = self._workspace("gram_i8", self.lib.effq_gram_i8_ws_bytes(C.byref(geom), int(ncls)))
        Au = Bu = None
        if unweighted:
            if acc:
                raise _lib.EffqError("gram_i8: the unweighted system is not accumulated across calls here")
            Au = torch.empty(n, n, dtype=torch.float64, device=self.device)
            Bu = torch.empty(geom.C2, n, dtype=torch.float64, device=self.device)
        check(self.lib.effq_gram_accum_i8_unw(_ptr(xidx_ndhwc), _ptr(y), C.byref(geom), int(has_bias), _ptr(al),
                                              int(act_levels), _ptr(lst), _ptr(chunk_cls), _ptr(cls_w), int(ncls),
                                              0 if lst is None else int(lst.numel()), _ptr(A0), _ptr(B0), acc,
                                              _ptr(Au), _ptr(Bu), _ptr(ws), ws.numel(), self.stream),
              "effq_gram_accum_i8_unw")
        return (A0, B0, Au, Bu) if unweighted else (A0, B0)

    def gram_f64_supported(self, geom: Geom, has_bias: bool) -> bool:
        return bool(self.lib.effq_gram_f64_supported(C.byref(geom), int(has_bias)))

    def gram_f64(self, x_ndhwc: torch.Tensor, y_ndhwc: torch.Tensor, geom: Geom, has_bias: bool):
        x, y = self._f32(x_ndhwc), self._f32(y_ndhwc)
        _check_shapes(geom, x, y=y)
        n = geom.C1 * geom.KD * geom.KH * geom.KW + int(has_bias)
        Au = torch.empty(n, n, dtype=torch.float64, device=self.device)
        Bu = torch.empty(geom.C2, n, dtype=torch.float64, device=self.device)
        ws = self._workspace("gram_f64", self.lib.effq_gram_f64_ws_bytes(C.byref(geom), int(has_bias)))
        check(self.lib.effq_gram_f64(_ptr(x), _ptr(y), C.byref(geom), int(has_bias), _ptr(Au), _ptr(Bu), _ptr(ws),
                                     ws.numel(), self.stream), "effq_gram_f64")
        return Au, Bu

    def upsample_trilinear(self, x_ndhwc: torch.Tensor, scale) -> torch.Tensor:
        x = self._f32(x_ndhwc)
        N, D, H, W, Cc = (int(i) for i in x.shape)
        sd, sh, sw = (int(i) for i in scale)
        out = torch.empty(N, D * sd, H * sh, W * sw, Cc, dtype=torch.float32, device=self.device)
        check(self.lib.effq_upsample_trilinear(_ptr(x), N, D, H, W, Cc, sd, sh, sw, _ptr(out), self.stream),
              "effq_upsample_trilinear")
        return out

    def gram_loss(self, Au: torch.Tensor, Bu: torch.Tensor, syy: torch.Tensor, G: torch.Tensor, b, sqerr=None):
        c2, n = (int(i) for i in Bu.shape)
        has_b = b is not None
        if (Au.dtype != torch.float64 or Bu.dtype != torch.float64 or syy.dtype != torch.float64 or
                tuple(Au.shape) != (n, n) or G.numel() != c2 * (n - int(has_b))):
            raise _lib.EffqError("gram_loss: operand shapes / dtypes do not match")
        if sqerr is None:
            sqerr = torch.zeros(2, dtype=torch.float64, device=self.device)
        ws = self._workspace("gram_loss", self.lib.effq_gram_loss_ws_bytes(n))
        check(self.lib.effq_gram_loss(_ptr(Au), _ptr(Bu), _ptr(syy), _ptr(self._f32(G)), _ptr(b), c2, n, int(has_b),
                                      _ptr(sqerr), _ptr(ws), ws.numel(), self.stream), "effq_gram_loss")
        return sqerr

    def gram_loss_i8_supported(self, c2: int, n: int, has_b: bool, w_levels: int) -> bool:
        return bool(self.lib.effq_gram_loss_i8_supported(int(c2), int(n), int(has_b), int(w_levels)))

    def gram_loss_i8_planes(self, Au: torch.Tensor, has_b: bool, act_alpha: torch.Tensor, act_levels: int, voxels: int):
        n = int(Au.shape[0])
        P = self.lib.effq_gram_loss_i8_num_planes(int((act_levels - 1) ** 2 * voxels))
        if P < 1:
            return None
        nw = n - int(has_b)
        planes = torch.empty(P, (nw + 255) // 256 * 256, nw, dtype=torch.int8, device=self.device)
        assert planes.numel() == self.lib.effq_gram_loss_i8_planes_bytes(n, int(has_b), P)
        err = torch.zeros(1, dtype=torch.int32, device=self.device)
        al = self._f32(act_alpha.reshape(1))
        check(self.lib.effq_gram_loss_i8_prepare(_ptr(Au), n, int(has_b), _ptr(al), int(act_levels), P, _ptr(planes),
                                                 _ptr(err), self.stream), "effq_gram_loss_i8_prepare")
        planes._effq_err = err
        return planes

    def gram_loss_i8(self, planes, Au, Bu, syy, Gq, b, states, act_alpha, act_levels: int, w_levels: int, hist=None):
        count, c2 = int(Gq.shape[0]), int(Bu.shape[0])
        n = int(Bu.shape[1])
        has_b = b is not None
        if hist is None:
            hist = torch.zeros(count, 2, dtype=torch.float64, device=self.device)
        ws = self._workspace("gram_loss_i8", self.lib.effq_gram_loss_i8_ws_bytes())
        al = self._f32(act_alpha.reshape(1))
        check(self.lib.effq_gram_loss_i8(_ptr(planes), int(planes.shape[0]), _ptr(Au), _ptr(Bu), _ptr(syy), _ptr(Gq), _ptr(b),
                                         _ptr(states), _ptr(al), int(act_levels), int(w_levels), c2, n, int(has_b), count,
                                         _ptr(hist), _ptr(ws), ws.numel(), self.stream), "effq_gram_loss_i8")
        return hist

    def gram_reduce(self, A0: torch.Tensor, B0: torch.Tensor, reducer):
        n, c2 = int(A0.shape[0]), int(B0.shape[0])
        buf = torch.empty(self.lib.effq_gram_packed_elems(n, c2), dtype=torch.float32, device=self.device)
        check(self.lib.effq_gram_pack(_ptr(A0), _ptr(B0), n, c2, _ptr(buf), self.stream), "effq_gram_pack")
        reducer(buf)
        check(self.lib.effq_gram_unpack(_ptr(buf), n, c2, _ptr(A0), _ptr(B0), self.stream), "effq_gram_unpack")
        return A0, B0

    @staticmethod
    def storage_bits(levels: int) -> int:
        for b in (1, 2, 4, 8):
            if levels <= (1 << b):
                return b
        raise _lib.EffqError(f"{levels} levels do not fit 8 bits")

    def pack_levels(self, idx: torch.Tensor, bits: int) -> torch.Tensor:
        if idx.dtype != torch.uint8 or not idx.is_contiguous():
            raise _lib.EffqError("pack_levels wants contiguous uint8 level ids")
        nb = self.lib.effq_packed_bytes(idx.numel(), int(bits))
        if idx.numel() and nb == 0:
            raise _lib.EffqError(f"unsupported field width {bits}")
        out = torch.empty(int(nb), dtype=torch.uint8, device=idx.device)
        check(self.lib.effq_pack_levels(_ptr(idx), idx.numel(), int(bits), _ptr(out), self.stream), "effq_pack_levels")
        return out

    def unpack_levels(self, packed: torch.Tensor, n: int, bits: int) -> torch.Tensor:
        if packed.dtype != torch.uint8 or packed.numel() != self.lib.effq_packed_bytes(int(n), int(bits)):
            raise _lib.EffqError("unpack_levels: buffer does not match n and the field width")
        out = torch.empty(int(n), dtype=torch.uint8, device=packed.device)
        check(self.lib.effq_unpack_levels(_ptr(packed.contiguous()), int(n), int(bits), _ptr(out), self.stream),
              "effq_unpack_levels")
        return out

    def spd_inverse(self, A0: torch.Tensor, has_bias: bool, rho: float, eta: float,
                    out: Optional[torch.Tensor] = None, ws_key: str = "inv") -> torch.Tensor:
        n = A0.shape[0]
        A0 = self._f32(A0)
        if out is None:
            out = torch.empty(n, self.lib.effq_ainv_ld(n), dtype=torch.float32, device=self.device)
        ws = self._workspace(ws_key, self.lib.effq_spd_inverse_ws_bytes(n))
        check(self.lib.effq_spd_inverse(_ptr(A0), n, int(has_bias), rho, eta, _ptr(out), _ptr(ws), ws.numel(),
                                        self.stream), "effq_spd_inverse")
        return out

    def spd_inverse_plan(self, n: int) -> dict:
        wide, nblk, piv = C.c_int(), C.c_int(), C.c_int()
        check(self.lib.effq_spd_inverse_plan(int(n), C.byref(wide), C.byref(nblk), C.byref(piv)), "effq_spd_inverse_plan")
        return dict(wide=bool(wide.value), nblk=nblk.value, pivot_blocks=piv.value)

    def prox_plan(self, c2: int, n: int) -> dict:
        v, gx, gy, ns = C.c_int(), C.c_int(), C.c_int(), C.c_int()
        check(self.lib.effq_prox_plan_query(int(c2), int(n), C.byref(v), C.byref(gx), C.byref(gy), C.byref(ns)),
              "effq_prox_plan_query")
        return dict(variant=v.value, gx=gx.value, gy=gy.value, nsplit=ns.value)

    def prox_solve(self, B0, Ainv, W0, b0, G, dual, rho: float, eta: float, wstar, bstar):
        c2, n = B0.shape
        ws = self._workspace("prox", self.lib.effq_prox_ws_bytes(c2, n))
        check(self.lib.effq_prox_solve(_ptr(B0), _ptr(Ainv), _ptr(W0), _ptr(b0), _ptr(G), _ptr(dual), c2, n,
                                       int(b0 is not None), rho, eta, _ptr(wstar), _ptr(bstar), _ptr(ws),
                                       ws.numel(), self.stream), "effq_prox_solve")

    PROX_SHIFT_TERMS = 26

    def prox_solve_shifted(self, B0, Ainv, W0, b0, G, dual, rho: float, eta: float, rho_inv: float, wstar, bstar):
        c2, n = B0.shape
        ws = self._workspace("prox", self.lib.effq_prox_ws_bytes(c2, n))
        terms = self.shift_terms(rho, eta, rho_inv)
        check(self.lib.effq_prox_solve_shifted(_ptr(B0), _ptr(Ainv), _ptr(W0), _ptr(b0), _ptr(G), _ptr(dual), c2, n,
                                               int(b0 is not None), rho, eta, rho_inv, terms, _ptr(wstar),
                                               _ptr(bstar), _ptr(ws), ws.numel(), self.stream),
              "effq_prox_solve_shifted")

    def admm_run(self, A0, B0, W0, b0, geom: Geom, y_ndhwc, *, xq=None, xidx=None, act_alpha=None, act_levels: int = 0,
                 loss_kind: int = 0, rho: float, rho_max: float, eta: float, iters: int, period: int, levels: int,
                 overlap: bool = True, loss_gram=None, residuals: bool = False, channel_wise: bool = False):
        from types import SimpleNamespace
        c2, n = (int(i) for i in B0.shape)
        has_b = b0 is not None
        W0, A0, B0 = self._f32(W0), self._f32(A0), self._f32(B0)
        b0 = self._f32(b0) if has_b else None
        xq = self._f32(xq) if xq is not None else None
        nw = W0.numel()
        y = self._f32(y_ndhwc)
        planes = None
        if loss_gram is not None and len(loss_gram) == 4:
            loss_kind = 5
            planes = loss_gram[3]
            loss_gram = loss_gram[:3]
        elif loss_gram is not None:
            loss_kind = 4
        if channel_wise and loss_kind not in (0, 4):
            raise _lib.EffqError(f"admm_run: channel mode takes loss kinds 0 and 4, not {loss_kind}")
        _check_shapes(geom, xq if loss_kind in (0, 4, 5) else xidx, W0, b0, y)
        if tuple(A0.shape) != (n, n) or nw != c2 * (n - int(has_b)):
            raise _lib.EffqError("admm_run: A0/B0/W0 shapes do not match")
        n_inv = self.lib.effq_admm_num_inverses(float(rho), float(rho_max), int(iters), int(period))
        if n_inv < 1:
            raise _lib.EffqError("admm_run: bad rho schedule")
        dev, f32 = self.device, torch.float32
        ld = self.lib.effq_ainv_ld(n)
        r = SimpleNamespace(iters=int(iters), nw=nw, c2=c2, has_b=has_b, channel_wise=bool(channel_wise))
        r.ainv = torch.empty(n_inv, n, ld, dtype=f32, device=dev)
        r.dual = torch.empty(nw, dtype=f32, device=dev)
        r.wstar = torch.empty(nw, dtype=f32, device=dev)
        r.v = torch.empty(nw, dtype=f32, device=dev)
        r.G_ring = torch.empty(iters, nw, dtype=f32, device=dev)
        r.Gq_ring = torch.empty(iters, nw, dtype=torch.int8, device=dev) if loss_kind in (1, 2, 5) else None
        r.b_ring = torch.empty(iters, c2, dtype=f32, device=dev) if has_b else None
        r.state_ring = torch.zeros(iters, 5, dtype=torch.float64, device=dev)
        r.hist = torch.zeros(iters, 2, dtype=torch.float64, device=dev)
        r.err = torch.zeros(1, dtype=torch.int32, device=dev)
        r.res = torch.zeros(iters, 2, dtype=torch.float64, device=dev) if residuals else None
        r.alpha_ring = torch.zeros(iters, c2, dtype=torch.float64, device=dev) if channel_wise else None
        r.w_iters_ring = torch.zeros(iters, c2, dtype=torch.int32, device=dev) if channel_wise else None
        main = torch.cuda.current_stream(dev)
        loss_s = self.loss_stream() if overlap else None
        side_s = self.side_stream()
        prox = self._workspace("prox", self.lib.effq_prox_ws_bytes(c2, n))
        inv = self._workspace("inv", self.lib.effq_spd_inverse_ws_bytes(n))
        inv_side = (self._workspace("inv_side", self.lib.effq_spd_inverse_ws_bytes(n))
                    if n_inv > 1 else None)
        inv_side2 = (self._workspace("inv_side2", self.lib.effq_spd_inverse_ws_bytes(n))
                     if n_inv > 2 else None)
        fpw = (self._workspace("fp_bucket", self.lib.effq_fp_bucket_ws_bytes(nw))
               if nw <= self.lib.effq_fp_bucket_max() and not channel_wise else None)
        traj = not channel_wise and bool(self.lib.effq_admm_uses_traj(nw, int(levels)))
        tws = self._workspace("fp_traj", self.lib.effq_fp_traj_ws_bytes(nw)) if traj else None
        r.fp_pred = torch.zeros(self.lib.effq_fp_traj_pred_bytes(), dtype=torch.uint8, device=dev) if traj else None
        if loss_kind == 5:
            cws = self._workspace("gram_loss_i8", self.lib.effq_gram_loss_i8_ws_bytes())
        elif loss_kind == 4:
            cws = self._workspace("gram_loss", self.lib.effq_gram_loss_ws_bytes(n))
        elif loss_kind == 1:
            cws = self._workspace("conv_i8", self.lib.effq_conv_i8_ws_bytes(C.byref(geom)))
        elif loss_kind == 2:
            cws = self._workspace("conv_i8s", self.lib.effq_conv_i8s_ws_bytes(C.byref(geom), int(act_levels),
                                                                             int(levels)))
        else:
            cws = self._workspace("conv", self.lib.effq_conv_ws_bytes(C.byref(geom)))
        al = self._f32(act_alpha.reshape(1)) if (act_alpha is not None and loss_kind in (1, 2, 5)) else None
        a = _lib.AdmmRunArgs()
        p = lambda t: None if t is None else t.data_ptr()
        a.A0, a.B0, a.W0, a.b0 = p(A0), p(B0), p(W0), p(b0)
        a.c2, a.n, a.has_bias, a.w_levels = c2, n, int(has_b), int(levels)
        a.iters, a.rho_period = int(iters), int(period)
        a.rho, a.rho_max, a.eta, a.tol = float(rho), float(rho_max), float(eta), ADMM_TOL
        a.geom = geom
        a.loss_kind, a.act_levels = int(loss_kind), int(act_levels)
        a.xq = p(xq) if loss_kind == 0 else None
        a.xidx = p(xidx) if loss_kind in (1, 2) else None
        if loss_kind in (4, 5):
            Au, Bu, syy = loss_gram
            if (Au.dtype != torch.float64 or Bu.dtype != torch.float64 or syy.dtype != torch.float64 or
                    tuple(Au.shape) != (n, n) or tuple(Bu.shape) != (c2, n) or syy.numel() != 1):
                raise _lib.EffqError("admm_run: loss_gram wants fp64 (Au [n,n], Bu [c2,n], syy [1])")
            a.loss_Au, a.loss_Bu, a.loss_syy = p(Au), p(Bu), p(syy)
            if loss_kind == 5:
                a.loss_planes, a.loss_nplanes = p(planes), int(planes.shape[0])
                r.loss_planes = planes
        a.y_fp, a.act_alpha_dev = p(y), p(al)
        a.dual, a.wstar, a.v = p(r.dual), p(r.wstar), p(r.v)
        a.G_ring, a.Gq_ring, a.b_ring = p(r.G_ring), p(r.Gq_ring), p(r.b_ring)
        a.state_ring, a.hist, a.err_flag = p(r.state_ring), p(r.hist), p(r.err)
        a.res_ring = p(r.res)
        a.channel_wise, a.alpha_ring, a.w_iters_ring = int(bool(channel_wise)), p(r.alpha_ring), p(r.w_iters_ring)
        a.ainv_pool, a.n_ainv = p(r.ainv), n_inv
        a.prox_ws, a.prox_ws_bytes = p(prox), prox.numel()
        a.red_ws = p(self._red_ws)
        a.fp_ws, a.fp_ws_bytes = p(fpw), (fpw.numel() if fpw is not None else 0)
        a.fp_pred, a.fp_traj_ws, a.fp_traj_ws_bytes = p(r.fp_pred), p(tws), (tws.numel() if tws is not None else 0)
        a.inv_ws, a.inv_ws_bytes = p(inv), inv.numel()
        a.inv_ws_side, a.inv_ws_side_bytes = p(inv_side), (inv_side.numel() if inv_side is not None else 0)
        a.conv_ws, a.conv_ws_bytes = p(cws), cws.numel()
        a.stream_main = main.cuda_stream
        a.stream_loss = loss_s.cuda_stream if loss_s is not None else None
        a.stream_side = side_s.cuda_stream if inv_side is not None else None
        if inv_side2 is not None:
            a.stream_side2 = self.side_stream2().cuda_stream
            a.inv_ws_side2, a.inv_ws_side2_bytes = p(inv_side2), inv_side2.numel()
        r.keep = (A0, B0, W0, b0, y, xq, xidx, al, loss_gram)
        check(self.lib.effq_admm_run(C.byref(a)), "effq_admm_run")
        return r

    def admm_select_best(self, run):
        best_G = torch.empty(run.nw, dtype=torch.float32, device=self.device)
        best_b = torch.empty(run.c2, dtype=torch.float32, device=self.device) if run.has_b else None
        best = torch.empty(2, dtype=torch.float64, device=self.device)
        check(self.lib.effq_admm_select_best(_ptr(run.hist), run.iters, _ptr(run.G_ring), _ptr(run.b_ring), run.nw,
                                             run.c2, _ptr(best_G), _ptr(best_b), _ptr(best), self.stream),
              "effq_admm_select_best")
        return best_G, best_b, best

    @staticmethod
    def admm_read(run, best, extra=None):
        err = run.err.to(torch.float64)
        if getattr(run, "loss_planes", None) is not None:
            err = err + 1000.0 * run.loss_planes._effq_err.to(torch.float64)
        if getattr(run, "channel_wise", False):
            return HipOps._admm_read_channels(run, best, err, extra)
        parts = [run.hist[:, 0], best, run.state_ring[-1, :1], run.state_ring[:, 4], err]
        if extra is not None:
            parts.append(extra.to(torch.float64).reshape(-1))
        pack = torch.cat(parts).cpu()
        it = run.iters
        w_iters = pack[it + 3: 2 * it + 3].contiguous().view(torch.int32)[0::2].tolist()
        return dict(hist=pack[:it].tolist(), best=pack[it:it + 2].tolist(), alpha_w=float(pack[it + 2]),
                    w_iters=w_iters, err=int(pack[2 * it + 3]),
                    extra=pack[2 * it + 4:].tolist() if extra is not None else None)

    @staticmethod
    def channel_alpha_best(run, best):
        return run.alpha_ring.index_select(0, best[1:2].to(torch.long)).reshape(-1)

    @staticmethod
    def _admm_read_channels(run, best, err, extra):
        it, c2 = run.iters, run.c2
        wmax, wrow = run.w_iters_ring.max(dim=1)
        parts = [run.hist[:, 0], best, HipOps.channel_alpha_best(run, best), wmax.to(torch.float64),
                 wrow.to(torch.float64), err]
        if extra is not None:
            parts.append(extra.to(torch.float64).reshape(-1))
        pack = torch.cat(parts).cpu()
        o = it + 2
        a_w = pack[o:o + c2].tolist()
        o += c2
        w_iters = [int(v) for v in pack[o:o + it].tolist()]
        w_rows = [int(v) for v in pack[o + it:o + 2 * it].tolist()]
        o += 2 * it
        return dict(hist=pack[:it].tolist(), best=pack[it:it + 2].tolist(), alpha_w=a_w, w_iters=w_iters,
                    w_iters_rows=w_rows, err=int(pack[o]), extra=pack[o + 1:].tolist() if extra is not None else None)

    def fixed_point_channels(self, a, b, v, levels: int, alpha, iters=None, err_flag=None, proj=None):
        c2 = int(a.shape[0])
        nwrow = a.numel() // c2
        tol, cap = ADMM_TOL, 100 * int(levels)
        if proj is None:
            check(self.lib.effq_fixed_point_channels(_ptr(a), _ptr(b), _ptr(v), c2, nwrow, int(levels), tol, cap,
                                                     _ptr(alpha), _ptr(iters), _ptr(err_flag), self.stream),
                  "effq_fixed_point_channels")
            return
        Bm = proj.get("Bm")
        B0 = proj.get("B0")
        check(self.lib.effq_fixed_point_channels_proj(
            _ptr(a), _ptr(b), _ptr(v), c2, nwrow, int(levels), tol, cap, _ptr(alpha), _ptr(iters), _ptr(err_flag),
            _ptr(proj["G"]), float(proj["dual_div"]), _ptr(Bm), _ptr(B0), _ptr(proj.get("W0")),
            int(B0.shape[1]) if B0 is not None else 0, int(proj.get("ldb", 0)), float(proj.get("rho_next", 0.0)),
            float(proj.get("eta", 0.0)), self.stream), "effq_fixed_point_channels_proj")

    def shift_terms(self, rho: float, eta: float, rho_inv: float) -> int:
        d = rho_inv - rho
        return 1 if d <= 0 else min(64, max(2, int(math.ceil(-26.0 * math.log(2.0) / math.log(d / (rho_inv + eta))))))

    def admm_presum(self, wstar, dual, v):
        check(self.lib.effq_admm_presum(_ptr(wstar), _ptr(dual), _ptr(v), wstar.numel(), self.stream),
              "effq_admm_presum")

    def admm_project_dual(self, v, wstar, state, levels: int, G, dual, dual_div: float, Gq=None):
        check(self.lib.effq_admm_project_dual(_ptr(v), _ptr(wstar), _ptr(state), levels, _ptr(G), _ptr(dual),
                                              float(dual_div), _ptr(Gq), v.numel(), self.stream),
              "effq_admm_project_dual")

    def conv_i8_supported(self, geom: Geom, act_levels: int, w_levels: int) -> bool:
        return bool(self.lib.effq_conv_i8_supported(C.byref(geom), int(act_levels), int(w_levels)))

    def conv_i8s_supported(self, geom: Geom, act_levels: int, w_levels: int) -> bool:
        return bool(self.lib.effq_conv_i8s_supported(C.byref(geom), int(act_levels), int(w_levels)))

    def conv_step_i8s(self, xidx: torch.Tensor, Gq: torch.Tensor, bias, geom: Geom, y_ndhwc: torch.Tensor,
                      act_alpha: torch.Tensor, act_levels: int, w_state: torch.Tensor, w_levels: int, sqerr,
                      prepare: bool):
        if xidx.dtype != torch.uint8 or Gq.dtype != torch.int8:
            raise _lib.EffqError("conv_step_i8s wants uint8 level ids and int8 weight operands")
        _check_shapes(geom, xidx, Gq, bias, y_ndhwc)
        al = self._f32(act_alpha.reshape(1))
        ws = self._workspace("conv_i8s", self.lib.effq_conv_i8s_ws_bytes(C.byref(geom), int(act_levels), int(w_levels)))
        check(self.lib.conv3d_calib_step_i8s(_ptr(xidx), _ptr(Gq), _ptr(bias), _ptr(self._f32(y_ndhwc)),
                                             C.byref(geom), _ptr(al), int(act_levels), _ptr(w_state), int(w_levels),
                                             int(bool(prepare)), _ptr(sqerr), _ptr(ws), ws.numel(), self.stream),
              "conv3d_calib_step_i8s")
        return sqerr

    def conv_step_i8(self, xidx: torch.Tensor, Gq: torch.Tensor, bias, geom: Geom, y_ndhwc: torch.Tensor,
                     act_alpha: torch.Tensor, act_levels: int, w_state: torch.Tensor, w_levels: int, sqerr):
        if xidx.dtype != torch.uint8 or Gq.dtype != torch.int8:
            raise _lib.EffqError("conv_step_i8 wants uint8 level ids and int8 weight numerators")
        _check_shapes(geom, xidx, Gq, bias, y_ndhwc)
        al = self._f32(act_alpha.reshape(1))
        ws = self._workspace("conv_i8", self.lib.effq_conv_i8_ws_bytes(C.byref(geom)))
        check(self.lib.conv3d_calib_step_i8(_ptr(xidx), _ptr(Gq), _ptr(bias), _ptr(self._f32(y_ndhwc)), C.byref(geom),
                                            _ptr(al), int(act_levels), _ptr(w_state), int(w_levels), _ptr(sqerr),
                                            _ptr(ws), ws.numel(), self.stream), "conv3d_calib_step_i8")
        return sqerr

    def conv_i8_out_supported(self, geom: Geom, act_levels: int, w_levels: int) -> bool:
        return bool(self.lib.effq_conv_i8_out_supported(C.byref(geom), int(act_levels), int(w_levels)))

    def conv_forward_i8(self, xidx: torch.Tensor, G: torch.Tensor, bias, geom: Geom, y_ndhwc: torch.Tensor, att,
                        act_alpha: torch.Tensor, act_levels: int, w_state: torch.Tensor, w_levels: int):
        if xidx.dtype != torch.uint8:
            raise _lib.EffqError("conv_forward_i8 wants uint8 level ids")
        att_f = self._f32(att) if att is not None else None
        _check_shapes(geom, xidx, G, bias, y_ndhwc, att_f)
        lm1 = int(w_levels) - 1
        a32 = w_state.reshape(-1)[0].to(torch.float32)
        Gq = (2.0 * torch.round((self._f32(G) / a32 + 1.0) * (0.5 * lm1)) - lm1).to(torch.int8).contiguous()
        al = self._f32(act_alpha.reshape(1))
        y = self._f32(y_ndhwc)
        out = torch.empty_like(y)
        sq = torch.zeros(2, dtype=torch.float64, device=self.device)
        st = w_state.to(torch.float64).contiguous()
        ws = self._workspace("conv_i8", self.lib.effq_conv_i8_ws_bytes(C.byref(geom)))
        check(self.lib.conv3d_quant_forward_i8(_ptr(xidx), _ptr(Gq), _ptr(self._f32(bias) if bias is not None else None),
                                               _ptr(y), _ptr(att_f), C.byref(geom), _ptr(al), int(act_levels), _ptr(st),
                                               int(w_levels), _ptr(sq), _ptr(out), _ptr(ws), ws.numel(), self.stream),
              "conv3d_quant_forward_i8")
        self._keep_i8 = (Gq, st, att_f, al)
        return out, sq

    def act_quant_backward(self, x: torch.Tensor, alpha: torch.Tensor, levels: int, gq: torch.Tensor, want_gx=True):
        x, gq = self._f32(x), self._f32(gq)
        a = self._f32(alpha.reshape(1))
        gx = torch.empty_like(x) if want_gx else None
        ga = torch.empty(1, dtype=torch.float64, device=self.device)
        check(self.lib.effq_act_quant_backward(_ptr(x), _ptr(a), int(levels), _ptr(gq), _ptr(gx), _ptr(ga), x.numel(),
                                               _ptr(self._red_ws), self.stream), "effq_act_quant_backward")
        return gx, ga

    def adam_step(self, p, g, m, v, lr: float, t: int, b1=0.9, b2=0.999, eps=1e-8):
        check(self.lib.effq_adam_step(_ptr(p), _ptr(g), _ptr(m), _ptr(v), lr, b1, b2, eps, int(t), p.numel(),
                                      self.stream), "effq_adam_step")

    def conv_step(self, x_ndhwc: torch.Tensor, weight: torch.Tensor, bias: Optional[torch.Tensor], geom: Geom,
                  y_ndhwc: Optional[torch.Tensor] = None, att: Optional[torch.Tensor] = None,
                  act_alpha: Optional[torch.Tensor] = None, act_levels: int = 0, want_out: bool = False,
                  sqerr: Optional[torch.Tensor] = None):
        x = self._f32(x_ndhwc)
        w = self._f32(weight)
        b = self._f32(bias) if bias is not None else None
        y = self._f32(y_ndhwc) if y_ndhwc is not None else None
        a = self._f32(att) if att is not None else None
        _check_shapes(geom, x, w, b, y, a)
        od, oh, ow = geom.out_dims()
        out = torch.empty(geom.N, od, oh, ow, geom.C2, dtype=torch.float32, device=self.device) if want_out else None
        if y is not None and sqerr is None:
            sqerr = torch.empty(2, dtype=torch.float64, device=self.device)
        al = self._f32(act_alpha.reshape(1)) if act_alpha is not None else None
        ws = self._workspace("conv", self.lib.effq_conv_ws_bytes(C.byref(geom)))
        check(self.lib.conv3d_quant_calib_step(_ptr(x), _ptr(w), _ptr(b), _ptr(y), _ptr(a), C.byref(geom), _ptr(al),
                                               int(act_levels), _ptr(sqerr), _ptr(out), _ptr(ws), ws.numel(),
                                               self.stream), "conv3d_quant_calib_step")
        return out, sqerr

    @staticmethod
    def window_grid(dhw, patch, overlap) -> Tuple[int, int, int]:
        n = []
        for s, p, o in zip(dhw, _triple(patch), _triple(overlap)):
            if p <= 0 or p > s:
                raise _lib.EffqError(f"window extent {p} outside 1..{s}")
            if o < 0 or o >= p:
                raise _lib.EffqError(f"overlap {o} must lie in 0..{p - 1}")
            n.append(len(range(0, s - p, p - o)) + 1)
        return tuple(n)

    def window_gather(self, vol: torch.Tensor, patch, overlap, first: int = 0, count: Optional[int] = None):
        x = self._f32(vol)
        if x.dim() != 5:
            raise _lib.EffqError(f"window_gather: expected N x C x D x H x W, got {tuple(x.shape)}")
        N, Cc, D, H, W = (int(i) for i in x.shape)
        p, o = _triple(patch), _triple(overlap)
        nwin = math.prod(self.window_grid((D, H, W), p, o))
        count = nwin - first if count is None else int(count)
        if first < 0 or count <= 0 or first + count > nwin:
            raise _lib.EffqError(f"windows {first}..{first + count - 1} of {nwin}")
        out = torch.empty(count * N, p[0], p[1], p[2], Cc, dtype=torch.float32, device=self.device)
        check(self.lib.effq_window_gather(_ptr(x), N, Cc, D, H, W, p[0], p[1], p[2], o[0], o[1], o[2], int(first), count,
                                          _ptr(out), self.stream), "effq_window_gather")
        return out

    def window_stitch(self, win: torch.Tensor, shape, patch, overlap) -> torch.Tensor:
        w = self._f32(win)
        N, Cc, D, H, W = (int(i) for i in shape)
        p, o = _triple(patch), _triple(overlap)
        nwin = math.prod(self.window_grid((D, H, W), p, o))
        if tuple(w.shape) != (nwin * N, p[0], p[1], p[2], Cc):
            raise _lib.EffqError(f"window_stitch: windows {tuple(w.shape)}, geometry needs {(nwin * N, *p, Cc)}")
        if not 0 < Cc <= 8:
            raise _lib.EffqError(f"window_stitch: {Cc} channels, at most 8")
        out = torch.empty(N, Cc, D, H, W, dtype=torch.float32, device=self.device)
        check(self.lib.effq_window_stitch(_ptr(w), N, Cc, D, H, W, p[0], p[1], p[2], o[0], o[1], o[2], _ptr(out),
                                          self.stream), "effq_window_stitch")
        return out

    def sigmoid_threshold(self) -> float:
        if getattr(self, "_sig_thresh", None) is not None:
            return self._sig_thresh

        def decide(mags):
            x = -torch.tensor(mags, dtype=torch.int32).view(torch.float32).to(self.device)
            return (torch.sigmoid(x) >= 0.5).cpu()

        lo, hi = 0, 0x3F800000
        while hi - lo > 1:
            cand = sorted({lo + (hi - lo) * k // 4097 for k in range(1, 4097)} - {lo, hi})
            ok = decide(cand)
            bad = (~ok).nonzero()
            first_bad = int(bad[0]) if len(bad) else len(cand)
            lo = cand[first_bad - 1] if first_bad > 0 else lo
            hi = cand[first_bad] if first_bad < len(cand) else hi
        dense = list(range(max(0, lo - (1 << 16)), lo + (1 << 16)))
        if not torch.equal(decide(dense), torch.tensor(dense) <= lo):
            raise _lib.EffqError("torch.sigmoid(x) >= 0.5 is not monotone around its threshold")
        self._sig_thresh = float(-torch.tensor([lo], dtype=torch.int32).view(torch.float32).item())
        return self._sig_thresh

    def _seg_case(self, what: str, logits: torch.Tensor, label: torch.Tensor, task: str, fuse, spatial: bool):
        x = self._f32(logits)
        if spatial and x.dim() != 4:
            raise _lib.EffqError(f"{what}: expected C x D x H x W logits, got {tuple(x.shape)}")
        Cc = int(x.shape[0])
        extents = tuple(int(i) for i in x.shape[1:]) if spatial else x[0].numel()
        if task == "lits":
            mode, lshape, thresh = _lib.SEG_ARGMAX, tuple(x.shape[1:]), 0.0
        elif task == "brats":
            mode, lshape, thresh = _lib.SEG_SIGMOID, tuple(x.shape), self.sigmoid_threshold()
        else:
            raise _lib.EffqError(f"Unknown task {task}")
        key = fuse.lower() if isinstance(fuse, str) else fuse
        if key not in _lib.SEG_FUSE or (mode == _lib.SEG_ARGMAX and key is not None):
            raise _lib.EffqError(f"{what}: merge type {fuse!r} for task {task}")
        if not 0 < Cc <= _lib.SEG_TALLIES_MAX_CLASSES:
            raise _lib.EffqError(f"{what}: {Cc} classes, at most {_lib.SEG_TALLIES_MAX_CLASSES}")
        if tuple(label.shape) != lshape or label.dtype != torch.uint8 or label.device != x.device:
            raise _lib.EffqError(f"{what}: label {tuple(label.shape)} {label.dtype} on {label.device}, "
                                 f"needs {lshape} torch.uint8 on {x.device}")
        return x, label.contiguous(), Cc, extents, mode, _lib.SEG_FUSE[key], thresh

    def _mask_planes(self, what: str, mask: torch.Tensor):
        if mask.dim() not in (3, 4) or mask.dtype != torch.uint8 or mask.numel() == 0:
            raise _lib.EffqError(f"{what}: mask {tuple(mask.shape)} {mask.dtype}, needs (P x) D x H x W torch.uint8")
        if mask.device != self.device and not (mask.device.type == "cuda" and
                                               self.device.index in (None, mask.device.index)):
            raise _lib.EffqError(f"{what}: mask on {mask.device}, ops on {self.device}")
        m = mask.contiguous()
        D, H, W = (int(i) for i in m.shape[-3:])
        return m, (int(m.shape[0]) if m.dim() == 4 else 1), D, H, W

    def seg_tallies(self, logits: torch.Tensor, label: torch.Tensor, task: str, fuse: Optional[str] = None):
        x, lab, Cc, S, mode, fcode, thresh = self._seg_case("seg_tallies", logits, label, task, fuse, False)
        counts = torch.empty(Cc, 4, dtype=torch.int64, device=self.device)
        ws = self._workspace("seg_tallies", _lib.SEG_TALLIES_WS_BYTES)
        check(self.lib.effq_seg_tallies(_ptr(x), _ptr(lab), Cc, S, mode, fcode, thresh, _ptr(counts), _ptr(ws), ws.numel(),
                                        self.stream), "effq_seg_tallies")
        return counts

    def seg_labels(self, logits: torch.Tensor, rule: str, fuse: Optional[str] = None, dtype=torch.uint8):
        x = self._f32(logits)
        if x.dim() < 3:
            raise _lib.EffqError(f"seg_labels: expected N x C x spatial logits, got {tuple(x.shape)}")
        N, Cc, S = int(x.shape[0]), int(x.shape[1]), math.prod(x.shape[2:])
        if rule not in _lib.SEG_LABEL_RULES:
            raise _lib.EffqError(f"seg_labels: unknown rule {rule!r} (one of {', '.join(_lib.SEG_LABEL_RULES)})")
        key = fuse.lower() if isinstance(fuse, str) else fuse
        if key not in _lib.SEG_FUSE or (rule == "argmax" and key is not None):
            raise _lib.EffqError(f"seg_labels: merge type {fuse!r} for rule {rule}")
        if not 0 < Cc <= _lib.SEG_TALLIES_MAX_CLASSES:
            raise _lib.EffqError(f"seg_labels: {Cc} classes, at most {_lib.SEG_TALLIES_MAX_CLASSES}")
        if rule == "brats" and Cc < 3:
            raise _lib.EffqError(f"seg_labels: the brats rule needs 3 channels or more, got {Cc}")
        if dtype not in (torch.uint8, torch.uint16) or (rule == "planes" and dtype != torch.uint8):
# ... 114 lines not shown
```

### include/effq_hip.h

```cpp
#ifndef EFFQ_HIP_H
#define EFFQ_HIP_H

#include <stddef.h>
#include <stdint.h>

#ifdef __cplusplus
extern "C" {
#endif

enum {
  EFFQ_OK = 0,
  EFFQ_ERR_ARG = 1,
  EFFQ_ERR_HIP = 2,
  EFFQ_ERR_WORKSPACE = 3,
  EFFQ_ERR_NO_DEVICE = 4,
  EFFQ_ERR_NOT_CONVERGED = 5
};

typedef struct effq_geom {
  int32_t N, C1, C2;
  int32_t D, H, W;
  int32_t KD, KH, KW;
  int32_t SD, SH, SW;
  int32_t PD, PH, PW;
} effq_geom;

const char* effq_last_error(void);
int effq_version(void);
int effq_device_count(int* count);

int effq_quant_dequant_f32(const float* x, const float* alpha_dev, float lo, float hi, int levels,
                           float* y_out, uint8_t* idx_out, size_t n, void* stream);

int effq_quant_dequant_f64path(const float* x, const double* alpha_dev, double lo, double hi, int levels,
                               float* y_out, float* b_out, uint8_t* idx_out, size_t n, void* stream);

size_t effq_reduce_ws_bytes(void);

int effq_abs_sum_f64(const float* x, size_t n, double* sums_out, void* ws, void* stream);

int effq_moments_f64(const float* x, size_t n, double* sums_out, void* ws, void* stream);

int effq_alpha_stats_f64(const float* x, const double* alpha_dev, double lo, double hi, int levels,
                         size_t n, double* sums_out, const int32_t* done_flag_dev, void* ws, void* stream);

typedef struct effq_fp_state {
  double alpha;
  double alpha_prev;
  double sums[2];
  int32_t iters;
  int32_t done;
} effq_fp_state;

int effq_fp_init(effq_fp_state* state_dev, const double* abs_sums_dev, void* stream);
int effq_fp_update(effq_fp_state* state_dev, double tol, int max_iter, void* stream);

int effq_alpha_fixed_point(const float* x, size_t n, int levels, double lo, double hi, double tol,
                           int max_iter, int n_iters, effq_fp_state* state_dev, void* ws, void* stream);

size_t effq_fp_small_max(void);
int effq_fixed_point_small(const float* a, const float* b, float* v_out, size_t n, int levels, double lo, double hi,
                           double tol, int max_iter, effq_fp_state* state_dev, void* stream);
size_t effq_fp_coop_max(void);
int effq_fixed_point_coop(const float* a, const float* b, float* v_out, size_t n, int levels, double lo, double hi,
                          double tol, int max_iter, effq_fp_state* state_dev, void* ws, void* stream);
int effq_fp_coop_set_spin_limit(unsigned int polls);
size_t effq_fp_bucket_max(void);
size_t effq_fp_bucket_ws_bytes(size_t n);
int effq_fixed_point_bucket(const float* a, const float* b, float* v_out, size_t n, int levels, double lo, double hi,
                            double tol, int max_iter, effq_fp_state* state_dev, void* ws, size_t ws_bytes,
                            void* stream);

size_t effq_fp_traj_max(void);
size_t effq_fp_traj_ws_bytes(size_t n);
size_t effq_fp_traj_pred_bytes(void);
int effq_fixed_point_traj(const float* a, const float* b, float* v_out, size_t n, int levels, double lo, double hi,
                          double tol, int max_iter, effq_fp_state* state_dev, void* pred_dev, void* ws, size_t ws_bytes,
                          void* stream);
int effq_fixed_point_bucket_rec(const float* a, const float* b, float* v_out, size_t n, int levels, double lo, double hi,
                                double tol, int max_iter, effq_fp_state* state_dev, void* ws, size_t ws_bytes,
                                void* pred_dev, void* stream);
int effq_fixed_point_coop_rec(const float* a, const float* b, float* v_out, size_t n, int levels, double lo, double hi,
                              double tol, int max_iter, effq_fp_state* state_dev, void* ws, void* pred_dev, void* stream);

size_t effq_fp_bracket_ws_bytes(size_t n);
int effq_fp_bracket_init(effq_fp_state* state_dev, const double* abs_sums_dev, size_t n, int levels, int list_first,
                         void* ws, size_t ws_bytes, void* stream);
int effq_fp_bracket_run(const float* x, size_t n, int levels, double lo, double hi, double tol, int max_iter, int n_iters,
                        effq_fp_state* state_dev, void* ws, void* stream);
int effq_fp_bracket_stats(const float* x, size_t n, int levels, double lo, double hi, effq_fp_state* state_dev, void* ws,
                          void* stream);
int effq_fp_bracket_update(size_t n, int levels, double lo, double hi, double tol, int max_iter,
                           effq_fp_state* state_dev, void* ws, void* stream);
size_t effq_fp_bracket_export_words(void);
int effq_fp_bracket_export(const void* ws, size_t n, long long* out, float* list_out, size_t list_cap, void* stream);
int effq_fp_bracket_import(const void* ws_src, size_t n_src, const long long* pack_dev, int world, size_t list_cap,
                           effq_fp_state* state_dev, void* ws_dst, size_t ws_dst_bytes, void* stream);
int effq_fp_bracket_rebase(effq_fp_state* state_dev, void* ws, size_t n, void* stream);
int effq_fp_channels_max_row(void);
int effq_fixed_point_channels(const float* a, const float* b, float* v_out, int c2, int nwrow, int levels, double tol,
                              int max_iter, double* alpha_out, int32_t* iters_out, int32_t* err_flag_dev, void* stream);
int effq_fixed_point_channels_proj(const float* wstar, float* dual, float* v_out, int c2, int nwrow, int levels,
                                   double tol, int max_iter, double* alpha_out, int32_t* iters_out, int32_t* err_flag_dev,
                                   float* G, float dual_div, float* Bm, const float* B0, const float* W0, int n, int ldb,
                                   double rho_next, double eta, void* stream);

int effq_fp_check(const effq_fp_state* state_dev, int32_t* err_flag_dev, void* stream);

size_t effq_gram_ws_bytes(const effq_geom* g, int has_bias);
int effq_gram_accum(const float* x_ndhwc, const float* att, const float* y_ndhwc, const effq_geom* g,
                    int has_bias, float* A0, float* B0, int accumulate, void* ws, size_t ws_bytes,
                    void* stream);
int effq_gram_plan_query(const effq_geom* g, int has_bias, int* vec, int* nb, int* npairs, int* nsplit,
                         long long* vox_per_split, int* fold, int* finish_blocks);

int effq_gram_i8_supported(const effq_geom* g, int act_levels);
size_t effq_gram_i8_ws_bytes(const effq_geom* g, int ncls);
int effq_gram_accum_i8(const uint8_t* xidx_ndhwc, const float* y_ndhwc, const effq_geom* g, int has_bias,
                       const float* act_alpha_dev, int act_levels, const int32_t* vox_list,
                       const int32_t* chunk_cls, const float* cls_w_dev, int ncls, long long n_list,
                       float* A0, float* B0, int accumulate, void* ws, size_t ws_bytes, void* stream);
int effq_gram_accum_i8_unw(const uint8_t* xidx_ndhwc, const float* y_ndhwc, const effq_geom* g, int has_bias,
                           const float* act_alpha_dev, int act_levels, const int32_t* vox_list, const int32_t* chunk_cls,
                           const float* cls_w_dev, int ncls, long long n_list, float* A0, float* B0, int accumulate,
                           double* Au, double* Bu, void* ws, size_t ws_bytes, void* stream);
int effq_gram_i8_plan_query(const effq_geom* g, int ncls, long long n_list, int* nb, int* nbx, int* npairs, int* nchunks,
                            int* cps, int* nsplit);

int effq_gram_f64_supported(const effq_geom* g, int has_bias);
size_t effq_gram_f64_ws_bytes(const effq_geom* g, int has_bias);
int effq_gram_f64(const float* x_ndhwc, const float* y_ndhwc, const effq_geom* g, int has_bias, double* Au, double* Bu,
                  void* ws, size_t ws_bytes, void* stream);
int effq_gram_f64_plan_query(const effq_geom* g, int has_bias, int* nchunk, int* grid, int* ntiles, int* tpw);

size_t effq_gram_loss_ws_bytes(int n);
int effq_gram_loss(const double* Au, const double* Bu, const double* syy_dev, const float* G, const float* b, int c2, int n,
                   int has_bias, double* sqerr_out, void* ws, size_t ws_bytes, void* stream);

int effq_gram_loss_i8_supported(int c2, int n, int has_bias, int w_levels);
int effq_gram_loss_i8_num_planes(long long kmax);
size_t effq_gram_loss_i8_planes_bytes(int n, int has_bias, int nplanes);
int effq_gram_loss_i8_prepare(const double* Au, int n, int has_bias, const float* act_alpha_dev, int act_levels,
                              int nplanes, int8_t* planes, int32_t* err_flag_dev, void* stream);
size_t effq_gram_loss_i8_ws_bytes(void);
int effq_gram_loss_i8(const int8_t* planes, int nplanes, const double* Au, const double* Bu, const double* syy_dev,
                      const int8_t* Gq, const float* b, const effq_fp_state* states, const float* act_alpha_dev,
                      int act_levels, int w_levels, int c2, int n, int has_bias, int count, double* hist_out, void* ws,
                      size_t ws_bytes, void* stream);


size_t effq_att_classes_ws_bytes(void);
int effq_att_classes(const float* att, long long V, int32_t* vox_list, int32_t* chunk_cls, float* cls_w_dev,
                     int32_t* info_host_out, void* ws, void* stream);

int effq_spd_inverse_prepare(void* stream);
int effq_ainv_ld(int n);
size_t effq_spd_inverse_ws_bytes(int n);
int effq_spd_inverse(const float* A0, int n, int has_bias, double rho, double eta, float* Ainv,
                     void* ws, size_t ws_bytes, void* stream);
int effq_spd_inverse_plan(int n, int* wide, int* nblk, int* pivot_blocks);

size_t effq_prox_ws_bytes(int c2, int n);
int effq_prox_solve(const float* B0, const float* Ainv, const float* W0, const float* b0, const float* G,
                    const float* dual, int c2, int n, int has_bias, double rho, double eta, float* wstar,
                    float* bstar, void* ws, size_t ws_bytes, void* stream);
int effq_prox_plan_query(int c2, int n, int* variant, int* gx, int* gy, int* nsplit);

int effq_prox_solve_shifted(const float* B0, const float* Ainv, const float* W0, const float* b0, const float* G,
                            const float* dual, int c2, int n, int has_bias, double rho, double eta,
                            double rho_inv, int nterms, float* wstar, float* bstar, void* ws, size_t ws_bytes,
                            void* stream);

int effq_admm_presum(const float* wstar, const float* dual, float* v, size_t n, void* stream);
int effq_admm_project_dual(const float* v, const float* wstar, const effq_fp_state* state_dev, int levels,
                           float* G, float* dual, float dual_div, int8_t* Gq_out, size_t n, void* stream);
size_t effq_conv_ws_bytes(const effq_geom* g);
int conv3d_quant_calib_step(const float* xq_ndhwc, const float* G, const float* bias, const float* y_fp,
                            const float* att, const effq_geom* g, const float* act_alpha_dev, int act_levels,
                            double* sqerr_out, float* out, void* ws, size_t ws_bytes, void* stream);

int effq_conv_i8_supported(const effq_geom* g, int act_levels, int w_levels);
size_t effq_conv_i8_ws_bytes(const effq_geom* g);
int conv3d_calib_step_i8(const uint8_t* xidx_ndhwc, const int8_t* Gq, const float* bias, const float* y_fp,
                         const effq_geom* g, const float* act_alpha_dev, int act_levels,
                         const effq_fp_state* w_state_dev, int w_levels, double* sqerr_out, void* ws,
                         size_t ws_bytes, void* stream);
int effq_conv_i8_out_supported(const effq_geom* g, int act_levels, int w_levels);
int conv3d_quant_forward_i8(const uint8_t* xidx_ndhwc, const int8_t* Gq, const float* bias, const float* y_fp,
                            const float* att, const effq_geom* g, const float* act_alpha_dev, int act_levels,
                            const effq_fp_state* w_state_dev, int w_levels, double* sqerr_out, float* out, void* ws,
                            size_t ws_bytes, void* stream);

int effq_conv_i8s_supported(const effq_geom* g, int act_levels, int w_levels);
size_t effq_conv_i8s_ws_bytes(const effq_geom* g, int act_levels, int w_levels);
int conv3d_calib_step_i8s(const uint8_t* xidx_ndhwc, const int8_t* Gq, const float* bias, const float* y_fp,
                          const effq_geom* g, const float* act_alpha_dev, int act_levels,
                          const effq_fp_state* w_state_dev, int w_levels, int prepare, double* sqerr_out,
                          void* ws, size_t ws_bytes, void* stream);

int effq_act_quant_backward(const float* x, const float* alpha_dev, int levels, const float* gq, float* gx_out,
                            double* galpha_out, size_t n, void* ws, void* stream);
int effq_adam_step(float* p, const float* g, float* m, float* v, float lr, float b1, float b2, float eps,
                   int t, size_t n, void* stream);

typedef struct effq_admm_run_args {
  const float* A0; const float* B0; const float* W0; const float* b0;
  int32_t c2, n, has_bias, w_levels;
  int32_t iters, rho_period;
  double rho, rho_max, eta, tol;
  effq_geom geom;
  int32_t loss_kind, act_levels;
  const float* xq; const uint8_t* xidx; const float* y_fp; const float* act_alpha_dev;
  float* dual; float* wstar; float* v;
  float* G_ring; int8_t* Gq_ring; float* b_ring; effq_fp_state* state_ring; double* hist;
  int32_t* err_flag;
  float* ainv_pool; int32_t n_ainv;
  void* prox_ws; size_t prox_ws_bytes;
  void* red_ws;
  void* fp_ws; size_t fp_ws_bytes;
  void* fp_pred; void* fp_traj_ws; size_t fp_traj_ws_bytes;
  void* inv_ws; size_t inv_ws_bytes;
  void* inv_ws_side; size_t inv_ws_side_bytes;
  void* conv_ws; size_t conv_ws_bytes;
  void* stream_main; void* stream_loss; void* stream_side;
  void* stream_side2; void* inv_ws_side2; size_t inv_ws_side2_bytes;
  const double* loss_Au; const double* loss_Bu; const double* loss_syy;
  const int8_t* loss_planes; int32_t loss_nplanes;
  double* res_ring;
  int32_t channel_wise;
  double* alpha_ring; int32_t* w_iters_ring;
} effq_admm_run_args;
int effq_admm_uses_traj(size_t nw, int w_levels);
int effq_admm_num_inverses(double rho, double rho_max, int iters, int rho_period);
int effq_admm_run(const effq_admm_run_args* a);
int effq_admm_select_best(const double* hist, int iters, const float* G_ring, const float* b_ring, size_t nw, size_t nb,
                          float* best_G, float* best_b, double* best_out, void* stream);

size_t effq_gram_packed_elems(int n, int c2);
int effq_gram_pack(const float* A0, const float* B0, int n, int c2, float* buf, void* stream);
int effq_gram_unpack(const float* buf, int n, int c2, float* A0, float* B0, void* stream);

typedef struct effq_prof_record {
  int32_t kind, iter, loss_kind, c2, n;
  effq_geom geom;
  float ms;
} effq_prof_record;
int effq_prof_enable(int every);
int effq_prof_count(void);
int effq_prof_read(int i, effq_prof_record* out);

int effq_upsample_trilinear(const float* x_ndhwc, int N, int D, int H, int W, int C, int sd, int sh, int sw,
                            float* y_ndhwc, void* stream);

size_t effq_packed_bytes(size_t n, int bits);
int effq_pack_levels(const uint8_t* idx, size_t n, int bits, uint8_t* packed, void* stream);
int effq_unpack_levels(const uint8_t* packed, size_t n, int bits, uint8_t* idx, void* stream);

#define EFFQ_SEG_TALLIES_MAX_CLASSES 8
#define EFFQ_SEG_TALLIES_WS_BYTES (1024 * 3 * EFFQ_SEG_TALLIES_MAX_CLASSES * 4)
enum { EFFQ_SEG_ARGMAX = 0, EFFQ_SEG_SIGMOID = 1 };
enum { EFFQ_SEG_FUSE_NONE = 0, EFFQ_SEG_FUSE_AGG = 1, EFFQ_SEG_FUSE_CON = 2 };
int effq_window_gather(const float* vol, int N, int C, int D, int H, int W, int pd, int ph, int pw, int od, int oh,
                       int ow, int first, int count, float* out, void* stream);
int effq_window_stitch(const float* win, int N, int C, int D, int H, int W, int pd, int ph, int pw, int od, int oh,
                       int ow, float* out, void* stream);
int effq_seg_tallies(const float* logits, const uint8_t* label, int C, long long S, int mode, int fuse, float thresh,
                     long long* counts, void* ws, size_t ws_bytes, void* stream);

#define EFFQ_SEG_LABEL_ARGMAX 0
#define EFFQ_SEG_LABEL_BRATS 1
#define EFFQ_SEG_LABEL_RANK 2
#define EFFQ_SEG_LABEL_PLANES 3
int effq_seg_labels(const float* logits, int N, int C, long long S, int rule, int fuse, float thresh, int out_bytes,
                    void* out, void* stream);

size_t effq_cc_ws_bytes(int P, int D, int H, int W);
int effq_cc_label(const uint8_t* masks, int P, int D, int H, int W, int connectivity, int32_t* labels,
                  long long* ncomp, void* ws, size_t ws_bytes, void* stream);
int effq_seg_lesions(const float* logits, const uint8_t* label, int C, int D, int H, int W, int mode, int fuse,
                     float thresh, int connectivity, long long* counts, void* ws, size_t ws_bytes, void* stream);

#define EFFQ_EDT_MAX_LINE 16382
size_t effq_surf_ws_bytes(int P, int D, int H, int W);
int effq_edt_sq(const uint8_t* masks, int P, int D, int H, int W, int32_t* sq, void* ws, size_t ws_bytes, void* stream);
int effq_seg_surface(const float* logits, const uint8_t* label, int C, int D, int H, int W, int mode, int fuse,
                     float thresh, long long* counts, double* sums, void* ws, size_t ws_bytes, void* stream);

#define EFFQ_EDT_MM_MAX_EXTENT 4096
size_t effq_surf_mm_ws_bytes(int P, int D, int H, int W);
int effq_edt_sq_mm(const uint8_t* masks, int P, int D, int H, int W, float wd, float wh, float ww, float* sq, void* ws,
                   size_t ws_bytes, void* stream);
int effq_seg_surface_mm(const float* logits, const uint8_t* label, int C, int D, int H, int W, int mode, int fuse,
                        float thresh, float wd, float wh, float ww, long long* counts, float* sq, double* sums, void* ws,
                        size_t ws_bytes, void* stream);

#ifdef __cplusplus
}
#endif
#endif
```

Baseline: 24.51.

## Pre-split Ainv into bf16x3 planes once per inverse for prox GEMM reuse

After each SPD inverse is computed, a new kernel splits Ainv into three swizzled bf16 planes and stores them in a per-rho pool. A new prox GEMM variant reads these pre-split planes directly instead of re-splitting the f32 Ainv tile inside every ADMM iteration. This removes repeated split3 work and halves the B-side LDS footprint, at the cost of extra memory for the plane pool and one extra split kernel per inverse.

```diff
diff --git a/efficientq_amd/_lib.py b/efficientq_amd/_lib.py
--- a/efficientq_amd/_lib.py
+++ b/efficientq_amd/_lib.py
@@ -62,7 +62,8 @@
                 ("stream_side2", C.c_void_p), ("inv_ws_side2", C.c_void_p), ("inv_ws_side2_bytes", C.c_size_t),
                 ("loss_Au", C.c_void_p), ("loss_Bu", C.c_void_p), ("loss_syy", C.c_void_p),
                 ("loss_planes", C.c_void_p), ("loss_nplanes", C.c_int32), ("res_ring", C.c_void_p),
-                ("channel_wise", C.c_int32), ("alpha_ring", C.c_void_p), ("w_iters_ring", C.c_void_p)]
+                ("channel_wise", C.c_int32), ("alpha_ring", C.c_void_p), ("w_iters_ring", C.c_void_p),
+                ("ainv_planes_pool", C.c_void_p), ("ainv_planes_bytes", C.c_size_t)]
 
 
 class ProfRecord(C.Structure):
@@ -155,6 +156,7 @@
     "effq_spd_inverse_plan": (_I, [_I, _IP, _IP, _IP]),
     "effq_prox_plan_query": (_I, [_I, _I, _IP, _IP, _IP, _IP]),
     "effq_prox_ws_bytes": (_SZ, [_I, _I]),
+    "effq_prox_planes_bytes": (_SZ, [_I]),
     "effq_prox_solve": (_I, [_P, _P, _P, _P, _P, _P, _I, _I, _I, _D, _D, _P, _P, _P, _SZ, _P]),
     "effq_prox_solve_shifted": (_I, [_P, _P, _P, _P, _P, _P, _I, _I, _I, _D, _D, _D, _I, _P, _P, _P, _SZ, _P]),
     "effq_admm_presum": (_I, [_P, _P, _P, _SZ, _P]),
@@ -185,6 +187,18 @@
     "effq_seg_surface_mm": (_I, [_P, _P, _I, _I, _I, _I, _I, _I, _F, _F, _F, _F, _P, _P, _P, _P, _SZ, _P]),
 }
 
+_PP = C.POINTER(C.c_void_p)
+INTERNAL_SIGNATURES = {
+    "effq_prox_takes_planes": (_I, [_I, _I]),
+    "effq_split_planes": (_I, [_P, _I, _I, _I, _P, _P]),
+    "effq_ainv_planes": (_I, [_P, _I, _P, _SZ, _P]),
+    "effq_prox_solve_prebuilt": (_I, [_P, _P, _P, _P, _P, _P, _I, _I, _I, _D, _D, _P, _P, _P, _SZ, _P]),
+    "effq_prox_solve_prebuilt_parts": (_I, [_P, _P, _P, _P, _P, _P, _I, _I, _I, _D, _D, _P, _P, _P, _SZ, _P, _PP, _IP,
+                                            _IP]),
+    "effq_prox_solve_planes": (_I, [_P, _P, _P, _P, _P, _P, _P, _I, _I, _I, _D, _D, _P, _P, _P, _SZ, _P, _I, _PP, _IP,
+                                    _IP]),
+}
+
 SEG_TALLIES_WS_BYTES = 1024 * 3 * 8 * 4
 SEG_TALLIES_MAX_CLASSES = 8
 SEG_ARGMAX, SEG_SIGMOID = 0, 1
@@ -205,9 +219,10 @@
         raise EffqError(f"{LIB_PATH} is missing: run `python -c 'import __graft_entry__ as g; g.build()'` "
                         f"or `make -C efficientq_amd/csrc` (there is no CPU fallback)")
     lib = C.CDLL(LIB_PATH)
-    for name, (res, args) in SIGNATURES.items():
-        fn = getattr(lib, name)
-        fn.restype, fn.argtypes = res, args
+    for table in (SIGNATURES, INTERNAL_SIGNATURES):
+        for name, (res, args) in table.items():
+            fn = getattr(lib, name)
+            fn.restype, fn.argtypes = res, args
     _lib = lib
     return lib
 
diff --git a/efficientq_amd/csrc/admm_run.hip b/efficientq_amd/csrc/admm_run.hip
--- a/efficientq_amd/csrc/admm_run.hip
+++ b/efficientq_amd/csrc/admm_run.hip
@@ -163,6 +163,7 @@
   RhoPlan rhos;
   int first, n_inv;
   size_t ainv_elems;
+  size_t planes_bytes;
   bool chan, bucket, traj;
   int traj_after;
   hipStream_t s_main, s_loss, s_side, s_side2;
@@ -219,6 +220,15 @@
   p->n_inv = p->rhos.count - p->first;
   EFFQ_CHECK_ARG(a->n_ainv >= p->n_inv);
   p->ainv_elems = (size_t)p->n * (size_t)effq_ainv_ld(p->n);
+  p->planes_bytes =
+      (a->ainv_planes_pool != nullptr && effq_prox_takes_planes(p->c2, p->n)) ? effq_prox_planes_bytes(p->n) : 0;
+  if (p->planes_bytes != 0) {
+    EFFQ_CHECK_ARG((reinterpret_cast<uintptr_t>(a->ainv_planes_pool) & 15) == 0);
+    if (a->ainv_planes_bytes < (size_t)p->n_inv * p->planes_bytes) {
+      set_error("admm_run: plane pool %zu < %zu", a->ainv_planes_bytes, (size_t)p->n_inv * p->planes_bytes);
+      return EFFQ_ERR_WORKSPACE;
+    }
+  }
   p->s_main = as_stream(a->stream_main);
   p->s_loss = a->stream_loss ? as_stream(a->stream_loss) : p->s_main;
   p->s_side = (a->stream_side && a->inv_ws_side) ? as_stream(a->stream_side) : p->s_main;
@@ -264,15 +274,25 @@
   }
 };
 
+static unsigned char* planes_of(const effq_admm_run_args* a, const AdmmPlan& p, int slot) {
+  return p.planes_bytes ? static_cast<unsigned char*>(a->ainv_planes_pool) + (size_t)slot * p.planes_bytes : nullptr;
+}
+static int enqueue_inverse(const effq_admm_run_args* a, const AdmmPlan& p, int slot, double rho, void* ws, size_t wsb,
+                           hipStream_t st) {
+  float* dst = a->ainv_pool + (size_t)slot * p.ainv_elems;
+  if (const int rc = effq_spd_inverse(a->A0, p.n, p.has_b, rho, a->eta, dst, ws, wsb, st); rc != EFFQ_OK) return rc;
+  if (p.planes_bytes == 0) return EFFQ_OK;
+  return effq_ainv_planes(dst, p.n, planes_of(a, p, slot), p.planes_bytes, st);
+}
+
 static int enqueue_later_inverses(const effq_admm_run_args* a, const AdmmPlan& p, EventPool& events, hipEvent_t* ev_inv) {
   for (int r = p.first + 1; r < p.rhos.count; ++r) {
-    float* dst = a->ainv_pool + (size_t)(r - p.first) * p.ainv_elems;
     const bool on2 = p.two_sides && ((r - p.first) % 2 == 0);
     hipStream_t sr = on2 ? p.s_side2 : p.s_side;
     void* ws = !p.fork_side ? a->inv_ws : (on2 ? a->inv_ws_side2 : a->inv_ws_side);
     const size_t wsb = !p.fork_side ? a->inv_ws_bytes : (on2 ? a->inv_ws_side2_bytes : a->inv_ws_side_bytes);
     ProfScope ps(g_prof_every > 0, PROF_INVERSE, -1 - r, a, sr);
-    const int rc = effq_spd_inverse(a->A0, p.n, p.has_b, p.rhos.rho[r], a->eta, dst, ws, wsb, sr);
+    const int rc = enqueue_inverse(a, p, r - p.first, p.rhos.rho[r], ws, wsb, sr);
     if (rc != EFFQ_OK) return rc;
     ps.close();
     if (p.fork_side) {
@@ -307,7 +327,15 @@
                   a->state_ring + i, nullptr, 1, 0};
 }
 
-static int enqueue_prox(const effq_admm_run_args* a, const AdmmPlan& p, AdmmIter* it, const float* Ainv, bool bm_ready) {
+static int enqueue_prox(const effq_admm_run_args* a, const AdmmPlan& p, AdmmIter* it, const float* Ainv,
+                        const void* planes, bool bm_ready) {
+  if (!it->use_shift && planes != nullptr) {
+    const bool parts = bm_ready && it->use_traj && p.c2 <= 512;
+    return effq_prox_solve_planes(a->B0, Ainv, planes, a->W0, a->b0, it->G_prev, a->dual, p.c2, p.n, p.has_b, it->rho,
+                                  a->eta, a->wstar, it->bstar, a->prox_ws, a->prox_ws_bytes, p.s_main, bm_ready ? 1 : 0,
+                                  parts ? &it->parts : nullptr, parts ? &it->parts_n : nullptr,
+                                  parts ? &it->parts_ld : nullptr);
+  }
   if (!it->use_shift && bm_ready && it->use_traj && p.c2 <= 512)
     return effq_prox_solve_prebuilt_parts(a->B0, Ainv, a->W0, a->b0, it->G_prev, a->dual, p.c2, p.n, p.has_b, it->rho,
                                           a->eta, a->wstar, it->bstar, a->prox_ws, a->prox_ws_bytes, p.s_main,
@@ -460,14 +488,14 @@
     if (p.two_sides) EFFQ_HIP(hipStreamWaitEvent(p.s_side2, ev_fork, 0));
   }
   ProfScope p_inv(g_prof_every > 0, PROF_INVERSE, -1, a, p.s_main);
-  if (const int rc = effq_spd_inverse(a->A0, p.n, p.has_b, p.rhos.rho[p.first], a->eta, a->ainv_pool, a->inv_ws,
-                                      a->inv_ws_bytes, p.s_main); rc != EFFQ_OK)
+  if (const int rc = enqueue_inverse(a, p, 0, p.rhos.rho[p.first], a->inv_ws, a->inv_ws_bytes, p.s_main); rc != EFFQ_OK)
     return rc;
   p_inv.close();
   if (p.fork_loss)
     for (int e = 0; e < LOSS_EVENTS; ++e) EFFQ_HIP(events.take(&ev_loss[e]));
   bool bm_ready = false;
   const float* Ainv = nullptr;
+  const void* planes = nullptr;
   int k = 0;
   int cur = -1;
   int loss_next = 0;
@@ -484,10 +512,11 @@
         p_wait.close();
       }
       Ainv = a->ainv_pool + (size_t)(k - p.first) * p.ainv_elems;
+      planes = planes_of(a, p, k - p.first);
       cur = k;
     }
     ProfScope p_prox(it.prof, PROF_PROX, i, a, p.s_main);
-    if (const int rc = enqueue_prox(a, p, &it, Ainv, bm_ready); rc != EFFQ_OK) return rc;
+    if (const int rc = enqueue_prox(a, p, &it, Ainv, planes, bm_ready); rc != EFFQ_OK) return rc;
     p_prox.close();
     if (const int rc = enqueue_fixed_point(a, p, it, &bm_ready); rc != EFFQ_OK) return rc;
     if (a->res_ring != nullptr) {
diff --git a/efficientq_amd/csrc/internal.h b/efficientq_amd/csrc/internal.h
--- a/efficientq_amd/csrc/internal.h
+++ b/efficientq_amd/csrc/internal.h
@@ -27,6 +27,14 @@
                                    float* bstar, void* ws, size_t ws_bytes, void* stream, const float** part_out,
                                    int* nsplit_out, int* ldp_out);
 
+int effq_prox_takes_planes(int c2, int n);
+int effq_split_planes(const float* src, int rows, int ld, int rows_pad, void* planes, void* stream);
+int effq_ainv_planes(const float* Ainv, int n, void* planes, size_t planes_bytes, void* stream);
+int effq_prox_solve_planes(const float* B0, const float* Ainv, const void* ainv_planes, const float* W0, const float* b0,
+                           const float* G, const float* dual, int c2, int n, int has_bias, double rho, double eta,
+                           float* wstar, float* bstar, void* ws, size_t ws_bytes, void* stream, int prebuilt,
+                           const float** part_out, int* nsplit_out, int* ldp_out);
+
 int effq_fixed_point_traj_parts(const float* part, int nsplit, int ldp, int c2, int nwrow, int has_bias, const float* dual,
                                 float* wstar_out, float* bstar_out, float* v_out, int levels, double lo, double hi, double tol,
                                 int max_iter, effq_fp_state* state_dev, void* pred_dev, void* ws, size_t ws_bytes,
diff --git a/efficientq_amd/csrc/solve.hip b/efficientq_amd/csrc/solve.hip
--- a/efficientq_amd/csrc/solve.hip
+++ b/efficientq_amd/csrc/solve.hip
@@ -961,6 +961,158 @@
     }
 }
 
+constexpr int B3P_ROWS = 256;
+
+static inline size_t b3p_bytes(int rows_pad, int ld) { return (size_t)(ld / B3_K) * 3 * rows_pad * B3_K * sizeof(__bf16); }
+
+__global__ __launch_bounds__(256) void k_split_planes(const float* __restrict__ src, int rows, int ld, int rows_pad,
+                                                      __bf16* __restrict__ planes) {
+  const int r = blockIdx.x * 32 + (threadIdx.x >> 3);
+  const int c = blockIdx.y * 64 + (threadIdx.x & 7) * 8;
+  if (c >= ld || r >= rows_pad) return;
+  f32x4 v0 = {0.f, 0.f, 0.f, 0.f}, v1 = {0.f, 0.f, 0.f, 0.f};
+  if (r < rows) {
+    v0 = *reinterpret_cast<const f32x4*>(src + (size_t)r * ld + c);
+    v1 = *reinterpret_cast<const f32x4*>(src + (size_t)r * ld + c + 4);
+  }
+  bf16x4 lo[3], hi[3];
+  split3(v0, lo[0], lo[1], lo[2]);
+  split3(v1, hi[0], hi[1], hi[2]);
+  const int kt = c / B3_K, half = (c >> 3) & 1;
+  __bf16* out = planes + ((size_t)kt * 3 * rows_pad + r) * B3_K + ((half ^ ((r >> 3) & 1)) * 8);
+#pragma unroll
+  for (int p = 0; p < 3; ++p)
+    *reinterpret_cast<bf16x8*>(out + (size_t)p * rows_pad * B3_K) =
+        __builtin_shufflevector(lo[p], hi[p], 0, 1, 2, 3, 4, 5, 6, 7);
+}
+
+template <int BM, int BN, int WM, int WN>
+__global__ __launch_bounds__(512) void k_prox_gemm_b3p(const float* __restrict__ Bm, int ldb,
+                                                       const __bf16* __restrict__ Apl, int apl_rows, int n, int c2,
+                                                       int has_bias, float* __restrict__ wstar, float* __restrict__ bstar,
+                                                       float* __restrict__ part, int ldp) {
+  __builtin_amdgcn_s_setprio(2);
+  constexpr int MT = BM / WM / 32, NT = BN / WN / 32;
+  constexpr int NA = BM * 4 / 512;
+  constexpr int NBS = 3 * BN * 2;
+  constexpr int NB = (NBS + 511) / 512;
+  constexpr int A_ELEMS = 3 * BM * B3_LD, STAGE = A_ELEMS + 3 * BN * B3_K;
+  static_assert(WM * WN == 8 && MT >= 1 && NT >= 1 && NA >= 1 && B3P_ROWS % BN == 0, "8 waves");
+  extern __shared__ __attribute__((aligned(16))) unsigned char b3_lds[];
+  __bf16* lds = reinterpret_cast<__bf16*>(b3_lds);
+  const int tid = threadIdx.x, lane = tid & 63, wid = tid >> 6;
+  const int li = lane & 31, lh = lane >> 5;
+  const int wm = wid / WN, wn = wid % WN;
+  const int row0 = blockIdx.y * BM, col0 = blockIdx.x * BN;
+
+  f32x16 acc[MT][NT];
+#pragma unroll
+  for (int m = 0; m < MT; ++m)
+#pragma unroll
+    for (int t = 0; t < NT; ++t)
+#pragma unroll
+      for (int r = 0; r < 16; ++r) acc[m][t][r] = 0.0f;
+
+  f32x4 ra[NA];
+  bf16x8 rb[NB];
+  const float* pa[NA];
+  const __bf16* pb[NB];
+#pragma unroll
+  for (int q = 0; q < NA; ++q) {
+    const int u = tid + q * 512, r = u >> 2, c4 = u & 3;
+    pa[q] = Bm + (size_t)(row0 + r) * ldb + c4 * 4;
+  }
+#pragma unroll
+  for (int q = 0; q < NB; ++q) {
+    const int s = (tid + q * 512 < NBS) ? tid + q * 512 : tid;
+    pb[q] = Apl + ((size_t)(s / (2 * BN)) * apl_rows + col0) * B3_K + (s % (2 * BN)) * 8;
+  }
+  const size_t tile_b = (size_t)3 * apl_rows * B3_K;
+#define EFFQ_B3P_FETCH(kt_)                                                         \
+  {                                                                                 \
+    _Pragma("unroll") for (int q = 0; q < NA; ++q)                                  \
+        ra[q] = *reinterpret_cast<const f32x4*>(pa[q] + (kt_) * B3_K);              \
+    _Pragma("unroll") for (int q = 0; q < NB; ++q)                                  \
+        rb[q] = *reinterpret_cast<const bf16x8*>(pb[q] + (size_t)(kt_) * tile_b);   \
+  }
+#define EFFQ_B3P_STORE(stage)                                                                       \
+  {                                                                                                 \
+    __bf16* As_ = lds + (stage) * STAGE;                                                            \
+    __bf16* Bs_ = As_ + A_ELEMS;                                                                    \
+    _Pragma("unroll") for (int q = 0; q < NA; ++q) {                                                \
+      const int u = tid + q * 512, off = (u >> 2) * B3_LD + (u & 3) * 4;                            \
+      bf16x4 p0, p1, p2;                                                                            \
+      split3(ra[q], p0, p1, p2);                                                                    \
+      *reinterpret_cast<bf16x4*>(&As_[off]) = p0;                                                   \
+      *reinterpret_cast<bf16x4*>(&As_[BM * B3_LD + off]) = p1;                                      \
+      *reinterpret_cast<bf16x4*>(&As_[2 * BM * B3_LD + off]) = p2;                                  \
+    }                                                                                               \
+    _Pragma("unroll") for (int q = 0; q < NB; ++q)                                                  \
+      if ((q + 1) * 512 <= NBS || tid + q * 512 < NBS)                                              \
+        *reinterpret_cast<bf16x8*>(&Bs_[(tid + q * 512) * 8]) = rb[q];                              \
+  }
+  const int nkt = ldb / B3_K;
+  const int kt0 = (int)(((long long)nkt * blockIdx.z) / gridDim.z);
+  const int nk = (int)(((long long)nkt * (blockIdx.z + 1)) / gridDim.z);
+  EFFQ_B3P_FETCH(kt0)
+  EFFQ_B3P_STORE(0)
+  EFFQ_B3P_FETCH(min(kt0 + 1, nk - 1))
+  lds_barrier();
+  const int sw = (li >> 3) & 1;
+  for (int kt = kt0; kt < nk; ++kt) {
+    const int st = (kt - kt0) & 1;
+    if (kt + 1 < nk) EFFQ_B3P_STORE(st ^ 1)
+    EFFQ_B3P_FETCH(min(kt + 2, nk - 1))
+    const __bf16* As = lds + st * STAGE;
+    const __bf16* Bs = As + A_ELEMS;
+    bf16x8 a[MT][3], b[NT][3];
+#pragma unroll
+    for (int m = 0; m < MT; ++m)
+#pragma unroll
+      for (int p = 0; p < 3; ++p)
+        a[m][p] = *reinterpret_cast<const bf16x8*>(&As[p * BM * B3_LD + ((wm * MT + m) * 32 + li) * B3_LD + 8 * lh]);
+#pragma unroll
+    for (int t = 0; t < NT; ++t)
+#pragma unroll
+      for (int p = 0; p < 3; ++p)
+        b[t][p] = *reinterpret_cast<const bf16x8*>(&Bs[p * BN * B3_K + ((wn * NT + t) * 32 + li) * B3_K + 8 * (lh ^ sw)]);
+#pragma unroll
+    for (int m = 0; m < MT; ++m)
+#pragma unroll
+      for (int t = 0; t < NT; ++t) {
+        acc[m][t] = __builtin_amdgcn_mfma_f32_32x32x16_bf16(a[m][0], b[t][2], acc[m][t], 0, 0, 0);
+        acc[m][t] = __builtin_amdgcn_mfma_f32_32x32x16_bf16(a[m][1], b[t][1], acc[m][t], 0, 0, 0);
+        acc[m][t] = __builtin_amdgcn_mfma_f32_32x32x16_bf16(a[m][2], b[t][0], acc[m][t], 0, 0, 0);
+        acc[m][t] = __builtin_amdgcn_mfma_f32_32x32x16_bf16(a[m][0], b[t][1], acc[m][t], 0, 0, 0);
+        acc[m][t] = __builtin_amdgcn_mfma_f32_32x32x16_bf16(a[m][1], b[t][0], acc[m][t], 0, 0, 0);
+        acc[m][t] = __builtin_amdgcn_mfma_f32_32x32x16_bf16(a[m][0], b[t][0], acc[m][t], 0, 0, 0);
+      }
+    lds_barrier();
+  }
+#undef EFFQ_B3P_FETCH
+#undef EFFQ_B3P_STORE
+  const int nw = n - has_bias;
+  float* P = (gridDim.z > 1) ? part + (size_t)blockIdx.z * c2 * ldp : nullptr;
+#pragma unroll
+  for (int m = 0; m < MT; ++m)
+#pragma unroll
+    for (int t = 0; t < NT; ++t) {
+      const int col = col0 + (wn * NT + t) * 32 + li;
+#pragma unroll
+      for (int r = 0; r < 16; ++r) {
+        const int row = row0 + (wm * MT + m) * 32 + (r & 3) + 8 * (r >> 2) + 4 * lh;
+        if (row < c2 && col < n) {
+          if (P != nullptr)
+            P[(size_t)row * ldp + col] = acc[m][t][r];
+          else if (col < nw)
+            wstar[(size_t)row * nw + col] = acc[m][t][r];
+          else
+            bstar[row] = acc[m][t][r];
+        }
+      }
+    }
+}
+
 __global__ __launch_bounds__(256) void k_prox_reduce(const float* __restrict__ part, int ldp, int nsplit, int c2, int n,
                                                      int has_bias, float* __restrict__ wstar, float* __restrict__ bstar) {
   const size_t tot = (size_t)c2 * ldp, stride = (size_t)gridDim.x * blockDim.x;
@@ -1233,7 +1385,7 @@
                            const float* dual, int c2, int n, int has_bias, double rho, double eta, double shift,
                            int nterms, float* wstar, float* bstar, void* ws, size_t ws_bytes, void* stream,
                            bool prebuilt = false, const float** part_out = nullptr, int* nsplit_out = nullptr,
-                           int* ldp_out = nullptr) {
+                           int* ldp_out = nullptr, const void* ainv_planes = nullptr) {
   EFFQ_CHECK_ARG(B0 && Ainv && W0 && G && dual && wstar && ws && c2 > 0 && n > 0 && nterms >= 1);
   EFFQ_CHECK_ARG(!has_bias || (b0 != nullptr && bstar != nullptr));
   if (ws_bytes < effq_prox_ws_bytes(c2, n)) {
@@ -1265,7 +1417,20 @@
 #define EFFQ_PROX_LAUNCH(MT, WM, WN, NTN)                                                                              \
   hipLaunchKernelGGL((k_prox_gemm<MT, WM, WN, NTN>), grid, dim3(256), 0, st, Bm, ldb, Ainv, lda, n, c2, has_bias ? 1 : 0, \
                      wstar, bstar, part, ldb)
-    if (pl.variant == 5 || pl.variant == 7) {
+    if ((pl.variant == 5 || pl.variant == 7) && ainv_planes != nullptr) {
+      const size_t lds5 = (size_t)2 * (3 * 256 * B3_LD + 3 * 256 * B3_K) * sizeof(__bf16);
+      const size_t lds7 = (size_t)2 * (3 * 128 * B3_LD + 3 * 128 * B3_K) * sizeof(__bf16);
+      const __bf16* apl = reinterpret_cast<const __bf16*>(ainv_planes);
+      const int apl_rows = round_up(n, B3P_ROWS);
+      EFFQ_HIP((raise_lds_limit<k_prox_gemm_b3p<256, 256, 4, 2>>(lds5)));
+      EFFQ_HIP((raise_lds_limit<k_prox_gemm_b3p<128, 128, 2, 4>>(lds7)));
+      if (pl.variant == 5)
+        hipLaunchKernelGGL((k_prox_gemm_b3p<256, 256, 4, 2>), grid, dim3(512), lds5, st, Bm, ldb, apl, apl_rows, n, c2,
+                           has_bias ? 1 : 0, wstar, bstar, part, ldb);
+      else
+        hipLaunchKernelGGL((k_prox_gemm_b3p<128, 128, 2, 4>), grid, dim3(512), lds7, st, Bm, ldb, apl, apl_rows, n, c2,
+                           has_bias ? 1 : 0, wstar, bstar, part, ldb);
+    } else if (pl.variant == 5 || pl.variant == 7) {
       const size_t lds5 = (size_t)2 * 3 * (256 + 256) * B3_LD * sizeof(__bf16);
       const size_t lds7 = (size_t)2 * 3 * (128 + 128) * B3_LD * sizeof(__bf16);
       EFFQ_HIP((raise_lds_limit<k_prox_gemm_b3<256, 256, 4, 2>>(lds5)));
@@ -1334,6 +1499,43 @@
                          stream, true, part_out, nsplit_out, ldp_out);
 }
 
+size_t effq_prox_planes_bytes(int n) {
+  return n > 0 ? b3p_bytes(round_up(n, B3P_ROWS), effq_ainv_ld(n)) : 0;
+}
+static bool prox_takes_planes(int c2, int n) {
+  const int v = prox_plan(c2, n).variant;
+  return v == 5 || v == 7;
+}
+
+int effq_split_planes(const float* src, int rows, int ld, int rows_pad, void* planes, void* stream) {
+  EFFQ_CHECK_ARG(src && planes && rows > 0 && ld > 0 && (ld % 32) == 0 && rows_pad >= rows && (rows_pad % 32) == 0);
+  EFFQ_CHECK_ARG((reinterpret_cast<uintptr_t>(src) & 15) == 0 && (reinterpret_cast<uintptr_t>(planes) & 15) == 0);
+  hipLaunchKernelGGL(k_split_planes, dim3((unsigned)(rows_pad / 32), (unsigned)((ld + 63) / 64)), dim3(256), 0,
+                     as_stream(stream), src, rows, ld, rows_pad, reinterpret_cast<__bf16*>(planes));
+  EFFQ_LAUNCH_CHECK();
+  return EFFQ_OK;
+}
+
+int effq_ainv_planes(const float* Ainv, int n, void* planes, size_t planes_bytes, void* stream) {
+  EFFQ_CHECK_ARG(n > 0);
+  if (planes_bytes < effq_prox_planes_bytes(n)) {
+    set_error("ainv_planes: %zu bytes < required %zu", planes_bytes, effq_prox_planes_bytes(n));
+    return EFFQ_ERR_WORKSPACE;
+  }
+  return effq_split_planes(Ainv, n, effq_ainv_ld(n), round_up(n, B3P_ROWS), planes, stream);
+}
+
+int effq_prox_solve_planes(const float* B0, const float* Ainv, const void* ainv_planes, const float* W0, const float* b0,
+                           const float* G, const float* dual, int c2, int n, int has_bias, double rho, double eta,
+                           float* wstar, float* bstar, void* ws, size_t ws_bytes, void* stream, int prebuilt,
+                           const float** part_out, int* nsplit_out, int* ldp_out) {
+  EFFQ_CHECK_ARG(ainv_planes != nullptr && c2 > 0 && n > 0 && prox_takes_planes(c2, n));
+  EFFQ_CHECK_ARG(part_out == nullptr || (prebuilt != 0 && nsplit_out && ldp_out));
+  return prox_solve_impl(B0, Ainv, W0, b0, G, dual, c2, n, has_bias, rho, eta, 0.0, 1, wstar, bstar, ws, ws_bytes,
+                         stream, prebuilt != 0, part_out, nsplit_out, ldp_out, ainv_planes);
+}
+int effq_prox_takes_planes(int c2, int n) { return (c2 > 0 && n > 0 && prox_takes_planes(c2, n)) ? 1 : 0; }
+
 int effq_prox_solve_shifted(const float* B0, const float* Ainv, const float* W0, const float* b0, const float* G,
                             const float* dual, int c2, int n, int has_bias, double rho, double eta, double rho_inv,
                             int nterms, float* wstar, float* bstar, void* ws, size_t ws_bytes, void* stream) {
diff --git a/efficientq_amd/hip_ops.py b/efficientq_amd/hip_ops.py
--- a/efficientq_amd/hip_ops.py
+++ b/efficientq_amd/hip_ops.py
@@ -574,6 +574,34 @@
                                        int(b0 is not None), rho, eta, _ptr(wstar), _ptr(bstar), _ptr(ws),
                                        ws.numel(), self.stream), "effq_prox_solve")
 
+    def split_planes(self, src: torch.Tensor, rows_pad: Optional[int] = None) -> torch.Tensor:
+        rows, ld = src.shape
+        rows_pad = (rows + 255) // 256 * 256 if rows_pad is None else int(rows_pad)
+        out = torch.empty(6 * rows_pad * ld, dtype=torch.uint8, device=self.device)
+        check(self.lib.effq_split_planes(_ptr(src), rows, ld, rows_pad, _ptr(out), self.stream), "effq_split_planes")
+        return out
+
+    def prox_gemm(self, B0, Ainv, W0, b0, G, dual, rho: float, eta: float, wstar, bstar, ws, *, planes=None,
+                  prebuilt: bool = False, parts: bool = False):
+        c2, n = B0.shape
+        part, ns, ldp = C.c_void_p(), C.c_int(1), C.c_int(0)
+        head = (_ptr(B0), _ptr(Ainv)) + ((_ptr(planes),) if planes is not None else ()) + (
+            _ptr(W0), _ptr(b0), _ptr(G), _ptr(dual), c2, n, int(b0 is not None), rho, eta, _ptr(wstar), _ptr(bstar),
+            _ptr(ws), ws.numel(), self.stream)
+        outs = (C.byref(part), C.byref(ns), C.byref(ldp))
+        if planes is not None:
+            rc = self.lib.effq_prox_solve_planes(*head, int(prebuilt), *(outs if parts else (None, None, None)))
+        elif parts:
+            rc = self.lib.effq_prox_solve_prebuilt_parts(*head, *outs)
+        elif prebuilt:
+            rc = self.lib.effq_prox_solve_prebuilt(*head)
+        else:
+            rc = self.lib.effq_prox_solve(*head)
+        check(rc, "prox_gemm")
+        if not parts:
+            return None
+        return (None if not part.value else (part.value - ws.data_ptr()) // 4), ns.value, ldp.value
+
     PROX_SHIFT_TERMS = 26
 
     def prox_solve_shifted(self, B0, Ainv, W0, b0, G, dual, rho: float, eta: float, rho_inv: float, wstar, bstar):
@@ -587,7 +615,8 @@
 
     def admm_run(self, A0, B0, W0, b0, geom: Geom, y_ndhwc, *, xq=None, xidx=None, act_alpha=None, act_levels: int = 0,
                  loss_kind: int = 0, rho: float, rho_max: float, eta: float, iters: int, period: int, levels: int,
-                 overlap: bool = True, loss_gram=None, residuals: bool = False, channel_wise: bool = False):
+                 overlap: bool = True, loss_gram=None, residuals: bool = False, channel_wise: bool = False,
+                 ainv_planes: bool = True):
         from types import SimpleNamespace
         c2, n = (int(i) for i in B0.shape)
         has_b = b0 is not None
@@ -615,6 +644,8 @@
         ld = self.lib.effq_ainv_ld(n)
         r = SimpleNamespace(iters=int(iters), nw=nw, c2=c2, has_b=has_b, channel_wise=bool(channel_wise))
         r.ainv = torch.empty(n_inv, n, ld, dtype=f32, device=dev)
+        r.ainv_planes = (torch.empty(n_inv, self.lib.effq_prox_planes_bytes(n), dtype=torch.uint8, device=dev)
+                         if ainv_planes and self.prox_plan(c2, n)["variant"] in (5, 7) else None)
         r.dual = torch.empty(nw, dtype=f32, device=dev)
         r.wstar = torch.empty(nw, dtype=f32, device=dev)
         r.v = torch.empty(nw, dtype=f32, device=dev)
@@ -679,6 +710,8 @@
         a.res_ring = p(r.res)
         a.channel_wise, a.alpha_ring, a.w_iters_ring = int(bool(channel_wise)), p(r.alpha_ring), p(r.w_iters_ring)
         a.ainv_pool, a.n_ainv = p(r.ainv), n_inv
+        a.ainv_planes_pool = p(r.ainv_planes)
+        a.ainv_planes_bytes = r.ainv_planes.numel() if r.ainv_planes is not None else 0
         a.prox_ws, a.prox_ws_bytes = p(prox), prox.numel()
         a.red_ws = p(self._red_ws)
         a.fp_ws, a.fp_ws_bytes = p(fpw), (fpw.numel() if fpw is not None else 0)
diff --git a/include/effq_hip.h b/include/effq_hip.h
--- a/include/effq_hip.h
+++ b/include/effq_hip.h
@@ -165,6 +165,7 @@
                     const float* dual, int c2, int n, int has_bias, double rho, double eta, float* wstar,
                     float* bstar, void* ws, size_t ws_bytes, void* stream);
 int effq_prox_plan_query(int c2, int n, int* variant, int* gx, int* gy, int* nsplit);
+size_t effq_prox_planes_bytes(int n);
 
 int effq_prox_solve_shifted(const float* B0, const float* Ainv, const float* W0, const float* b0, const float* G,
                             const float* dual, int c2, int n, int has_bias, double rho, double eta,
@@ -229,6 +230,7 @@
   double* res_ring;
   int32_t channel_wise;
   double* alpha_ring; int32_t* w_iters_ring;
+  void* ainv_planes_pool; size_t ainv_planes_bytes;
 } effq_admm_run_args;
 int effq_admm_uses_traj(size_t nw, int w_levels);
 int effq_admm_num_inverses(double rho, double rho_max, int iters, int rho_period);
```

Result: no change. 24.60 (median of 2 runs) (+0.4%).
